# eth-ait/MultiPly

Measured on AMD Instinct MI355X. Metric: rays/sec rendering full 512x512 frames (eval forward, all persons, with background), higher is better.
Workload: dtype f16; 1 GPU; 2-person synthetic SMPL scene, 512x512 rays/frame, N_samples=128 (+32 extra +2 bounds = 161 composited samples/ray/person), N_samples_eval=128, 32 background samples, convergence groups of 512 rays (reference pixel_per_batch), geometric-init weights; frames=32, persons=2, sampler_sdf=bf16x3, parallelism=single GPU

## Files before the change

### multiply_amd/csrc/mlp.hip

```cpp
#include <hip/hip_runtime.h>
#include "common.hpp"
#include "../../include/multiply_hip.h"
#include "mlp_core.hpp"

using namespace mp;

namespace {

static_assert(sizeof(MpNet) == sizeof(NetDesc), "host / device net descriptors must match");
static_assert(MP_BIAS_STRIDE == BIAS_STRIDE && MP_MAX_LAYERS == MAX_LAYERS && MP_MAX_CHUNKS == MAX_CHUNKS, "abi");

constexpr int BIAS_BYTES = MAX_LAYERS * BIAS_STRIDE * 4;

template <int KS_IN, int NB, int WAVES>
struct Lds {
    static constexpr int PTS = 16 * NB;
    static constexpr int TILE = PTS * WAVES;
    static constexpr int ring = 0;
    static constexpr int bias0 = RING_SLOTS * chunk_bytes(KS_IN);
    static constexpr int bias1 = bias0 + BIAS_BYTES;
    static constexpr int stage = bias1 + BIAS_BYTES;
    static constexpr int scratch = stage + WAVES * PTS * in_stride(KS_IN) * 2;
    static constexpr int total = scratch + WAVES * PTS * 16;
};

template <int D, int L, int KS_IN>
__device__ __forceinline__ void stage_pe(op_t* row, const float (&x)[D]) {
    constexpr int NF = D + 2 * D * L;
    static_assert(NF <= KS_IN * 32, "encoding does not fit the input K steps");
#pragma unroll
    for (int a = 0; a < D; ++a) row[a] = (op_t)x[a];
#pragma unroll
    for (int a = 0; a < D; ++a) {
        float s, c;
        sincosf(x[a], &s, &c);
#pragma unroll
        for (int k = 0; k < L; ++k) {
            row[D + 2 * D * k + a] = (op_t)s;
            row[D + 2 * D * k + D + a] = (op_t)c;
            const float s2 = 2.0f * s * c, c2 = 1.0f - 2.0f * s * s;
            s = s2;
            c = c2;
        }
    }
#pragma unroll
    for (int f = NF; f < KS_IN * 32; ++f) row[f] = (op_t)0.0f;
}

template <int L, int KS_IN>
__device__ __forceinline__ void stage_pe_tangent(op_t* row, const float (&x)[3], int axis) {
    constexpr int D = 3;
#pragma unroll
    for (int f = 0; f < KS_IN * 32; ++f) row[f] = (op_t)0.0f;
    float s, c;
    const float xa = axis == 0 ? x[0] : (axis == 1 ? x[1] : x[2]);
    sincosf(xa, &s, &c);
    row[axis] = (op_t)TANGENT_SCALE;
    float f = TANGENT_SCALE;
#pragma unroll
    for (int k = 0; k < L; ++k) {
        row[D + 2 * D * k + axis] = (op_t)(f * c);
        row[D + 2 * D * k + D + axis] = (op_t)(-f * s);
        const float s2 = 2.0f * s * c, c2 = 1.0f - 2.0f * s * s;
        s = s2;
        c = c2;
        f *= 2.0f;
    }
}

template <int NB>
__device__ __forceinline__ void zero_b(opx8 (&B)[KS_REG][NB]) {
#pragma unroll
    for (int k = 0; k < KS_REG; ++k)
#pragma unroll
        for (int nb = 0; nb < NB; ++nb) B[k][nb] = (opx8)(op_t)0.0f;
}

template <int NB, int WAVES>
__global__ __launch_bounds__(WAVES * 64) void k_mlp_sdf(const NetDesc net, const char* __restrict__ wpack,
                                                        const float* __restrict__ bias, const float* __restrict__ xc,
                                                        const int* __restrict__ worklist,
                                                        const int* __restrict__ count_p, int max_count,
                                                        float* __restrict__ sdf_out) {
    constexpr int KS_IN = 2;
    using L = Lds<KS_IN, NB, WAVES>;
    extern __shared__ __attribute__((aligned(16))) char smem[];
    const int wave = threadIdx.x >> 6, lane = threadIdx.x & 63;
    const int count = count_p ? min(*count_p, max_count) : max_count;
    float* bias_lds = (float*)(smem + L::bias0);
    op_t* stage = (op_t*)(smem + L::stage) + wave * L::PTS * in_stride(KS_IN);
    load_bias(net, bias, bias_lds);
    for (int t = blockIdx.x; t * L::TILE < count; t += gridDim.x) {
        MP_STAMP_AT(HID_SOFTPLUS, 120, 0);
        prologue_issue<KS_IN, WAVES>(net, wpack, smem + L::ring, wave, lane);
        const int w = t * L::TILE + wave * L::PTS + lane;
        const int id = (lane < L::PTS && w < count) ? (worklist ? worklist[w] : w) : -1;
        if (lane < L::PTS) {
            float x[3] = {0.f, 0.f, 0.f};
            if (id >= 0) { x[0] = xc[3 * (size_t)id]; x[1] = xc[3 * (size_t)id + 1]; x[2] = xc[3 * (size_t)id + 2]; }
            stage_pe<3, 6, KS_IN>(stage + lane * in_stride(KS_IN), x);
        }
        MP_STAMP_AT(HID_SOFTPLUS, 120, 1);
        opx8 Bcur[KS_REG][NB];
        f32x4 out[NB];
        zero_b<NB>(Bcur);
        prologue_wait();
        MP_STAMP_AT(HID_SOFTPLUS, 120, 2);
        run_net<NB, false, KS_IN, HID_SOFTPLUS, WAVES>(net, wpack, bias_lds, smem + L::ring, Bcur, stage, out, wave, lane);
        MP_STAMP_AT(HID_SOFTPLUS, 120, 3);
#pragma unroll
        for (int nb = 0; nb < NB; ++nb) {
            const int pid = __shfl(id, nb * 16 + (lane & 15));
            if (lane < 16 && pid >= 0) sdf_out[pid] = out[nb][0];
        }
        MP_STAMP_AT(HID_SOFTPLUS, 121, 0);
    }
}

template <int WAVES>
__global__ __launch_bounds__(WAVES * 64) void k_mlp_sdf_x2(const NetDesc net, const char* __restrict__ wpack,
                                                           const float* __restrict__ bias, const float* __restrict__ xc,
                                                           const int* __restrict__ worklist,
                                                           const int* __restrict__ count_p, int max_count,
                                                           float* __restrict__ sdf_out) {
    constexpr int KS_IN = 2, NB = 2, WPTS = 16, TILE = WPTS * WAVES;
    using L = Lds<KS_IN, NB, WAVES>;
    constexpr int NF = 39, STR = in_stride(KS_IN);
    extern __shared__ __attribute__((aligned(16))) char smem[];
    const int wave = threadIdx.x >> 6, lane = threadIdx.x & 63, j = lane & 15, g = lane >> 4;
    const int count = count_p ? min(*count_p, max_count) : max_count;
    float* bias_lds = (float*)(smem + L::bias0);
    op_t* stage = (op_t*)(smem + L::stage) + wave * L::PTS * STR;
    load_bias(net, bias, bias_lds);
    for (int t = blockIdx.x; t * TILE < count; t += gridDim.x) {
        prologue_issue<KS_IN, WAVES>(net, wpack, smem + L::ring, wave, lane);
        const int w = t * TILE + wave * WPTS + j;
        const int id = w < count ? (worklist ? worklist[w] : w) : -1;
        {
            op_t* rh = stage + j * STR;
            op_t* rl = stage + (16 + j) * STR;
            auto put = [&](int f, float v) {
                const op_t hi = (op_t)v;
                rh[f] = hi;
                rl[f] = (op_t)(v - (float)hi);
            };
            if (g < 3) {
                const float x = id >= 0 ? xc[3 * (size_t)id + g] : 0.0f;
                put(g, x);
#pragma unroll
                for (int k = 0; k < 6; ++k) {
                    float sn, cs;
                    sincosf(x * (float)(1 << k), &sn, &cs);
                    put(3 + 6 * k + g, sn);
                    put(3 + 6 * k + 3 + g, cs);
                }
            } else {
#pragma unroll
                for (int f = NF; f < KS_IN * 32; ++f) { rh[f] = (op_t)0.0f; rl[f] = (op_t)0.0f; }
            }
        }
        opx8 Bcur[KS_REG][NB];
        f32x4 out[NB];
        zero_b<NB>(Bcur);
        prologue_wait();
        run_net<NB, false, KS_IN, HID_SOFTPLUS_X2, WAVES>(net, wpack, bias_lds, smem + L::ring, Bcur, stage, out, wave, lane);
        if (lane < 16 && id >= 0) sdf_out[id] = out[0][0] + out[1][0];
    }
}

template <int D_IN, int LFREQ, int KS_IN, int NB, int WAVES>
__global__ __launch_bounds__(WAVES * 64) void k_mlp_full(const NetDesc net, const char* __restrict__ wpack,
                                                         const float* __restrict__ bias, const float* __restrict__ x,
                                                         int n, float* __restrict__ outp) {
    using L = Lds<KS_IN, NB, WAVES>;
    extern __shared__ __attribute__((aligned(16))) char smem[];
    const int wave = threadIdx.x >> 6, lane = threadIdx.x & 63;
    float* bias_lds = (float*)(smem + L::bias0);
    op_t* stage = (op_t*)(smem + L::stage) + wave * L::PTS * in_stride(KS_IN);
    load_bias(net, bias, bias_lds);
    for (int t = blockIdx.x; t * L::TILE < n; t += gridDim.x) {
        const int id0 = t * L::TILE + wave * L::PTS;
        if (lane < L::PTS) {
            const int id = id0 + lane < n ? id0 + lane : -1;
            float xi[D_IN];
#pragma unroll
            for (int a = 0; a < D_IN; ++a) xi[a] = id >= 0 ? x[(size_t)id * D_IN + a] : 0.f;
            stage_pe<D_IN, LFREQ, KS_IN>(stage + lane * in_stride(KS_IN), xi);
        }
        opx8 Bcur[KS_REG][NB];
        f32x4 out[NB];
        zero_b<NB>(Bcur);
        prologue<KS_IN, WAVES>(net, wpack, smem + L::ring, wave, lane);
        run_net<NB, false, KS_IN, HID_SOFTPLUS, WAVES>(net, wpack, bias_lds, smem + L::ring, Bcur, stage, out, wave, lane);
        const int j = lane & 15, g = lane >> 4;
#pragma unroll
        for (int nb = 0; nb < NB; ++nb) {
            const int pid = id0 + nb * 16 + j;
            if (pid < n) {
                float* o = outp + (size_t)pid * 257;
                if (g == 0) o[0] = out[nb][0];
#pragma unroll
                for (int ks = 0; ks < KS_REG; ++ks)
#pragma unroll
                    for (int e = 0; e < 8; ++e)
                        o[1 + 32 * ks + (e < 4 ? 4 * g + e : 16 + 4 * g + e - 4)] = (float)Bcur[ks][nb][e];
            }
        }
    }
}

__global__ __launch_bounds__(512) void k_mlp_shade(const NetDesc net, const char* __restrict__ wpack,
                                                   const float* __restrict__ bias, const float* __restrict__ xc,
                                                   const float* __restrict__ jinv, const int* __restrict__ worklist,
                                                   const int* __restrict__ count_p, int max_count,
                                                   float* __restrict__ sdf_out, float* __restrict__ normal_out,
                                                   char* __restrict__ feat_frag) {
    constexpr int KS_IN = 2, NB = 2, WAVES = 8;
    using L = Lds<KS_IN, NB, WAVES>;
    extern __shared__ __attribute__((aligned(16))) char smem[];
    const int wave = threadIdx.x >> 6, lane = threadIdx.x & 63;
    const int count = count_p ? min(*count_p, max_count) : max_count;
    float* bias_lds = (float*)(smem + L::bias0);
    op_t* stage = (op_t*)(smem + L::stage) + wave * L::PTS * in_stride(KS_IN);
    load_bias(net, bias, bias_lds);
    for (int t = blockIdx.x; t * 64 < count; t += gridDim.x) {
        const int pt = lane & 7, role = 2 * ((lane >> 4) & 1) + ((lane >> 3) & 1);
        const int w = t * 64 + wave * 8 + pt;
        const int id = w < count ? (worklist ? worklist[w] : w) : -1;
        if (lane < 32) {
            float x[3] = {0.f, 0.f, 0.f};
            if (id >= 0) { x[0] = xc[3 * (size_t)id]; x[1] = xc[3 * (size_t)id + 1]; x[2] = xc[3 * (size_t)id + 2]; }
            op_t* row = stage + lane * in_stride(KS_IN);
            if (role == 0) stage_pe<3, 6, KS_IN>(row, x);
            else stage_pe_tangent<6, KS_IN>(row, x, role - 1);
        }
        opx8 Bcur[KS_REG][NB];
        f32x4 out[NB];
        zero_b<NB>(Bcur);
        prologue<KS_IN, WAVES, false>(net, wpack, smem + L::ring, wave, lane);
        run_net<NB, true, KS_IN, HID_SOFTPLUS, WAVES>(net, wpack, bias_lds, smem + L::ring, Bcur, stage, out, wave, lane);
        if ((lane & 8) == 0) {
            const int lp = ((lane & 15) + 8 * (wave & 1)) + 16 * (lane >> 4);
#pragma unroll
            for (int ks = 0; ks < KS_REG; ++ks)
                *(opx8*)(feat_frag + (((size_t)t * KS_REG + ks) * 4 + (wave >> 1)) * 1024 + lp * 16) = Bcur[ks][0];
        }
        constexpr float TS_INV = 1.0f / TANGENT_SCALE;
        const float gx = TS_INV * __shfl(out[0][0], (lane & 7) + 8), gz = TS_INV * __shfl(out[1][0], (lane & 7) + 8);
        if (lane < 8 && id >= 0) {
            const float gy = TS_INV * out[1][0];
            const float* Ji = jinv + 9 * (size_t)id;
            float n0 = gx * Ji[0] + gy * Ji[3] + gz * Ji[6];
            float n1 = gx * Ji[1] + gy * Ji[4] + gz * Ji[7];
            float n2 = gx * Ji[2] + gy * Ji[5] + gz * Ji[8];
            float inv = 1.0f / fmaxf(sqrtf(n0 * n0 + n1 * n1 + n2 * n2), 1e-12f);
            n0 *= inv; n1 *= inv; n2 *= inv;
            inv = 1.0f / fmaxf(sqrtf(n0 * n0 + n1 * n1 + n2 * n2), 1e-6f);
            sdf_out[id] = out[0][0];
            normal_out[3 * (size_t)id] = n0 * inv;
            normal_out[3 * (size_t)id + 1] = n1 * inv;
            normal_out[3 * (size_t)id + 2] = n2 * inv;
        }
    }
}

struct GradCapture {
    const op_t* tab_a;
    const op_t* tab_b;
    float (&g)[2][3];
    template <int NB>
    __device__ __forceinline__ void operator()(int cid, int bi, const f32x4 (&acc)[NB]) const {
        const int lane = threadIdx.x & 63, j = lane & 15, gq = lane >> 4;
        const op_t* tab = cid == 1 ? tab_a : tab_b;
#pragma unroll
        for (int nb = 0; nb < 2; ++nb) {
            const op_t* tp = tab + (16 * nb + j) * 48 + 16 * bi + 4 * gq;
#pragma unroll
            for (int r = 0; r < 4; ++r) {
                const float v = acc[nb][r] * (float)tp[r];
                const int k = (bi + r) % 3;
                g[nb][0] += k == 0 ? v : 0.0f;
                g[nb][1] += k == 1 ? v : 0.0f;
                g[nb][2] += k == 2 ? v : 0.0f;
            }
        }
    }
    static __device__ __forceinline__ void unrotate(float (&g)[2][3]) {
        const int s = ((threadIdx.x & 63) >> 4) % 3;
#pragma unroll
        for (int nb = 0; nb < 2; ++nb) {
            const float a0 = g[nb][0], a1 = g[nb][1], a2 = g[nb][2];
            g[nb][0] = s == 0 ? a0 : (s == 1 ? a2 : a1);
            g[nb][1] = s == 0 ? a1 : (s == 1 ? a0 : a2);
            g[nb][2] = s == 0 ? a2 : (s == 1 ? a1 : a0);
        }
    }
};


template <int NB, int WAVES>
__global__ __launch_bounds__(WAVES * 64) void k_mlp_fwdsave(const NetDesc net, const char* __restrict__ wpack,
                                                            const float* __restrict__ bias, const float* __restrict__ xc,
                                                            const int* __restrict__ worklist,
                                                            const int* __restrict__ count_p, int max_count, int offset,
                                                            int seg, float* __restrict__ sdf_out,
                                                            char* __restrict__ feat_frag, char* __restrict__ sigbuf) {
    constexpr int KS_IN = 2;
    using L = Lds<KS_IN, NB, WAVES>;
    static_assert(L::PTS == 32 && WAVES == 8, "feature / sigmoid block addressing assumes 8 waves x 32 points");
    extern __shared__ __attribute__((aligned(16))) char smem[];
    const int wave = threadIdx.x >> 6, lane = threadIdx.x & 63;
    const int count = min(count_p ? min(*count_p, max_count) : max_count, offset + seg);
    if (offset >= count) return;
    float* bias_lds = (float*)(smem + L::bias0);
    op_t* stage = (op_t*)(smem + L::stage) + wave * L::PTS * in_stride(KS_IN);
    load_bias(net, bias, bias_lds);
    constexpr int SIG_LAYER = KS_REG * SIG_CHUNK_BYTES;
    for (int t = blockIdx.x; offset + t * L::TILE < count; t += gridDim.x) {
        prologue_issue<KS_IN, WAVES>(net, wpack, smem + L::ring, wave, lane);
        const int w = offset + t * L::TILE + wave * L::PTS + lane;
        const int id = (lane < L::PTS && w < count) ? (worklist ? worklist[w] : w) : -1;
        if (lane < L::PTS) {
            float x[3] = {0.f, 0.f, 0.f};
            if (id >= 0) { x[0] = xc[3 * (size_t)id]; x[1] = xc[3 * (size_t)id + 1]; x[2] = xc[3 * (size_t)id + 2]; }
            stage_pe<3, 6, KS_IN>(stage + lane * in_stride(KS_IN), x);
        }
        opx8 Bcur[KS_REG][NB];
        f32x4 out[NB];
        zero_b<NB>(Bcur);
        prologue_wait();
        MP_STAMP_AT(HID_SOFTPLUS_SAVE, 120, 2);
        #ifdef MP_EXP_SIGCACHED
        const SigIO sio = {sigbuf + ((size_t)(blockIdx.x) * WAVES + wave) * (size_t)(8 * SIG_LAYER), SIG_LAYER};
#else
        const SigIO sio = {sigbuf + ((size_t)t * WAVES + wave) * (size_t)(8 * SIG_LAYER), SIG_LAYER};
#endif
        run_net<NB, false, KS_IN, HID_SOFTPLUS_SAVE, WAVES>(net, wpack, bias_lds, smem + L::ring, Bcur, stage, out, wave, lane,
                                                            sio);
        MP_STAMP_AT(HID_SOFTPLUS_SAVE, 120, 3);
        const size_t tile = (size_t)(offset / 64) + (size_t)t * 4 + (wave >> 1);
#pragma unroll
        for (int nb = 0; nb < NB; ++nb) {
#pragma unroll
            for (int ks = 0; ks < KS_REG; ++ks)
                *(opx8*)(feat_frag + ((tile * KS_REG + ks) * 4 + (wave & 1) * 2 + nb) * 1024 + lane * 16) = Bcur[ks][nb];
            const int pid = __shfl(id, nb * 16 + (lane & 15));
            if (lane < 16 && pid >= 0) sdf_out[pid] = out[nb][0];
        }
    }
}

template <int NB, int WAVES>
__global__ __launch_bounds__(WAVES * 64) void k_mlp_grad(const NetDesc net, const char* __restrict__ wpack,
                                                         const op_t* __restrict__ w8_slots, const float* __restrict__ xc,
                                                         const float* __restrict__ jinv, const int* __restrict__ worklist,
                                                         const int* __restrict__ count_p, int max_count, int offset, int seg,
                                                         const char* __restrict__ sigbuf, const float* __restrict__ sdf_in,
                                                         float* __restrict__ normal_out) {
    constexpr int KS_IN = 0, PTS = 16 * NB, TILE = PTS * WAVES;
    static_assert(NB == 2 && WAVES == 8, "matches k_mlp_fwdsave's tile / wave / point addressing");
    constexpr int RING = RING_SLOTS * chunk_bytes(KS_IN);
    extern __shared__ __attribute__((aligned(16))) char smem[];
    const int wave = threadIdx.x >> 6, lane = threadIdx.x & 63, gq = lane >> 4;
    const int count = min(count_p ? min(*count_p, max_count) : max_count, offset + seg);
    if (offset >= count) return;
    op_t* w8 = (op_t*)(smem + RING);
    op_t* tabs = w8 + 256 + wave * (2 * PTS * 48);
    for (int i = threadIdx.x; i < 256; i += blockDim.x) w8[i] = w8_slots[i];
    constexpr int SIG_LAYER = KS_REG * SIG_CHUNK_BYTES;
    for (int t = blockIdx.x; offset + t * TILE < count; t += gridDim.x) {
        const int w = offset + t * TILE + wave * PTS + (lane & (PTS - 1));
        const int id = w < count ? (worklist ? worklist[w] : w) : -1;
        if (lane < PTS) {
            float x[3] = {0.f, 0.f, 0.f};
            if (id >= 0) { x[0] = xc[3 * (size_t)id]; x[1] = xc[3 * (size_t)id + 1]; x[2] = xc[3 * (size_t)id + 2]; }
            op_t* ta = tabs + lane * 48;
            op_t* tb = tabs + PTS * 48 + lane * 48;
#pragma unroll
            for (int f = 0; f < 48; ++f) { ta[f] = (op_t)0.0f; tb[f] = (op_t)0.0f; }
#pragma unroll
            for (int a = 0; a < 3; ++a) {
                ta[a] = (op_t)1.0f;
                float sn, cs, fr = 1.0f;
                sincosf(x[a], &sn, &cs);
#pragma unroll
                for (int k = 0; k < 6; ++k) {
                    ta[3 + 6 * k + a] = (op_t)(fr * cs);
                    ta[3 + 6 * k + 3 + a] = (op_t)(-fr * sn);
                    const float s2 = 2.0f * sn * cs, c2 = 1.0f - 2.0f * sn * sn;
                    sn = s2; cs = c2; fr *= 2.0f;
                }
            }
#pragma unroll
            for (int f = 0; f < 39; ++f) tb[9 + f] = ta[f];
        }
        #ifdef MP_EXP_SIGCACHED
        const SigIO sio = {const_cast<char*>(sigbuf) + ((size_t)(blockIdx.x) * WAVES + wave) * (size_t)(8 * SIG_LAYER), SIG_LAYER};
#else
        const SigIO sio = {const_cast<char*>(sigbuf) + ((size_t)t * WAVES + wave) * (size_t)(8 * SIG_LAYER), SIG_LAYER};
#endif
        opx8 Bcur[KS_REG][NB];
        __syncthreads();
#pragma unroll
        for (int ks = 0; ks < KS_REG; ++ks) {
            const opx8 wv = *(const opx8*)(w8 + ks * 32 + 8 * gq);
            if constexpr (SIG8) {
                const u32x4 pk = *(const u32x4*)(sio.base + (size_t)7 * SIG_LAYER + ks * 1024 + lane * 16);
                const opx8 wq = wv * (op_t)SIG_QINV_F;
#pragma unroll
                for (int nb = 0; nb < NB; ++nb) {
                    const unsigned d0 = nb == 0 ? pk.x : pk.z, d1 = nb == 0 ? pk.y : pk.w;
                    u32x4 h;
                    h.x = __builtin_amdgcn_perm(0x64646464u, d0, 0x04010400u);
                    h.y = __builtin_amdgcn_perm(0x64646464u, d0, 0x04030402u);
                    h.z = __builtin_amdgcn_perm(0x64646464u, d1, 0x04010400u);
                    h.w = __builtin_amdgcn_perm(0x64646464u, d1, 0x04030402u);
                    Bcur[ks][nb] = (__builtin_bit_cast(opx8, h) - (op_t)1024.0f) * wq;
                }
            } else {
#pragma unroll
                for (int nb = 0; nb < NB; ++nb)
                    Bcur[ks][nb] = *(const opx8*)(sio.base + (size_t)7 * SIG_LAYER + (ks * NB + nb) * 1024 + lane * 16) * wv;
            }
        }
        float g[2][3] = {{0.f, 0.f, 0.f}, {0.f, 0.f, 0.f}};
        f32x4 out[NB];
#ifdef MP_EXP_GRAD_OLD
        prologue<KS_IN, WAVES, false>(net, wpack, smem, wave, lane);
#else
        prologue<KS_IN, WAVES>(net, wpack, smem, wave, lane);
#endif
        MP_STAMP_AT(HID_SIGMUL, 120, 2);
        run_net<NB, false, KS_IN, HID_SIGMUL, WAVES, GradCapture>(net, wpack, nullptr, smem, Bcur, nullptr, out, wave, lane, sio,
                                                                   GradCapture{tabs, tabs + PTS * 48, g});
        MP_STAMP_AT(HID_SIGMUL, 120, 3);
        GradCapture::unrotate(g);
#pragma unroll
        for (int nb = 0; nb < NB; ++nb)
#pragma unroll
            for (int a = 0; a < 3; ++a) {
                g[nb][a] += __shfl_xor(g[nb][a], 16);
                g[nb][a] += __shfl_xor(g[nb][a], 32);
            }
#pragma unroll
        for (int nb = 0; nb < NB; ++nb) {
            const int pid = __shfl(id, nb * 16 + (lane & 15));
            if (lane < 16 && pid >= 0) {
                const float gx = g[nb][0], gy = g[nb][1], gz = g[nb][2];
                const float* Ji = jinv + 9 * (size_t)pid;
                float n0 = gx * Ji[0] + gy * Ji[3] + gz * Ji[6];
                float n1 = gx * Ji[1] + gy * Ji[4] + gz * Ji[7];
                float n2 = gx * Ji[2] + gy * Ji[5] + gz * Ji[8];
                float inv = 1.0f / fmaxf(sqrtf(n0 * n0 + n1 * n1 + n2 * n2), 1e-12f);
                n0 *= inv; n1 *= inv; n2 *= inv;
                inv = 1.0f / fmaxf(sqrtf(n0 * n0 + n1 * n1 + n2 * n2), 1e-6f);
                const float poison = 0.0f * sdf_in[pid];
                normal_out[3 * (size_t)pid] = n0 * inv + poison;
                normal_out[3 * (size_t)pid + 1] = n1 * inv + poison;
                normal_out[3 * (size_t)pid + 2] = n2 * inv + poison;
            }
        }
        __syncthreads();
    }
}

template <int NB, int WAVES>
__global__ __launch_bounds__(WAVES * 64) void k_mlp_color(const NetDesc net, const char* __restrict__ wpack,
                                                          const float* __restrict__ bias, const float* __restrict__ xc,
                                                          const float* __restrict__ normal,
                                                          const char* __restrict__ feat_frag,
                                                          const int* __restrict__ worklist,
                                                          const int* __restrict__ count_p, int max_count,
                                                          float* __restrict__ rgb_out) {
    constexpr int KS_IN = 2;
    using L = Lds<KS_IN, NB, WAVES>;
    static_assert(64 % L::PTS == 0, "a wave consumes a whole number of column blocks of one 64-item shade tile");
    extern __shared__ __attribute__((aligned(16))) char smem[];
    const int wave = threadIdx.x >> 6, lane = threadIdx.x & 63;
    const int count = count_p ? min(*count_p, max_count) : max_count;
    float* bias_lds = (float*)(smem + L::bias0);
    op_t* stage = (op_t*)(smem + L::stage) + wave * L::PTS * in_stride(KS_IN);
    load_bias(net, bias, bias_lds);
    for (int t = blockIdx.x; t * L::TILE < count; t += gridDim.x) {
        MP_STAMP_AT(HID_RELU, 120, 0);
        const int w0 = t * L::TILE + wave * L::PTS;
        const int tile = w0 / 64, nb0 = (w0 % 64) / 16;
        const int w = w0 + lane;
        const int id = (lane < L::PTS && w < count) ? (worklist ? worklist[w] : w) : -1;
        prologue_issue<KS_IN, WAVES>(net, wpack, smem + L::ring, wave, lane);
        opx8 Bcur[KS_REG][NB];
        const bool live = w0 < count;
#pragma unroll
        for (int ks = 0; ks < KS_REG; ++ks)
#pragma unroll
            for (int nb = 0; nb < NB; ++nb)
                Bcur[ks][nb] = live ? *(const opx8*)(feat_frag + (((size_t)tile * KS_REG + ks) * 4 + nb0 + nb) * 1024 + lane * 16)
                                    : (opx8)(op_t)0.0f;
        if (lane < L::PTS) {
            op_t* row = stage + lane * in_stride(KS_IN);
#pragma unroll
            for (int f = 0; f < KS_IN * 32; ++f) row[f] = (op_t)0.0f;
            if (id >= 0) {
#pragma unroll
                for (int a = 0; a < 3; ++a) {
                    row[a] = (op_t)xc[3 * (size_t)id + a];
                    row[3 + a] = (op_t)normal[3 * (size_t)id + a];
                }
            }
        }
        MP_STAMP_AT(HID_RELU, 120, 1);
        f32x4 out[NB];
        prologue_wait();
        MP_STAMP_AT(HID_RELU, 120, 2);
        run_net<NB, false, KS_IN, HID_RELU, WAVES>(net, wpack, bias_lds, smem + L::ring, Bcur, stage, out, wave, lane);
        MP_STAMP_AT(HID_RELU, 120, 3);
#pragma unroll
        for (int nb = 0; nb < NB; ++nb) {
            const int pid = __shfl(id, nb * 16 + (lane & 15));
            if (lane < 16 && pid >= 0) {
                const float* nq = normal + 3 * (size_t)pid;
                const float poison = 0.0f * (nq[0] + nq[1] + nq[2]);
#pragma unroll
                for (int c = 0; c < 3; ++c) rgb_out[3 * (size_t)pid + c] = 1.0f / (1.0f + __expf(-out[nb][c])) + poison;
            }
        }
        MP_STAMP_AT(HID_RELU, 121, 0);
    }
}

template <int NB, int WAVES>
__global__ __launch_bounds__(WAVES * 64) void k_background(const NetDesc net_imp, const char* __restrict__ wp_imp,
                                                           const float* __restrict__ bias_imp, const NetDesc net_ren,
                                                           const char* __restrict__ wp_ren,
                                                           const float* __restrict__ bias_ren,
                                                           const float* __restrict__ dirs, const float* __restrict__ cam,
                                                           const float* __restrict__ z_bg, int z_per_ray, int n_rays,
                                                           float radius, float* __restrict__ bg_rgb) {
    constexpr int KS_IN = 3, NBG = 32;
    using L = Lds<KS_IN, NB, WAVES>;
    static_assert(L::PTS % NBG == 0, "whole rays per wave");
    extern __shared__ __attribute__((aligned(16))) char smem[];
    const int wave = threadIdx.x >> 6, lane = threadIdx.x & 63;
    float* bias_lds0 = (float*)(smem + L::bias0);
    float* bias_lds1 = (float*)(smem + L::bias1);
    op_t* stage = (op_t*)(smem + L::stage) + wave * L::PTS * in_stride(KS_IN);
    float* scr = (float*)(smem + L::scratch) + wave * L::PTS * 4;
    load_bias(net_imp, bias_imp, bias_lds0);
    load_bias(net_ren, bias_ren, bias_lds1);
    const int n_pts = n_rays * NBG;
    const float ox = cam[0], oy = cam[1], oz = cam[2];
    for (int t = blockIdx.x; t * L::TILE < n_pts; t += gridDim.x) {
        prologue_issue<KS_IN, WAVES>(net_imp, wp_imp, smem + L::ring, wave, lane);
        const int q = t * L::TILE + wave * L::PTS + lane;
        const int ray = q / NBG, s = q % NBG;
        float d[3] = {0.f, 0.f, 1.f};
        if (lane < L::PTS) {
            const bool ok = ray < n_rays;
            float depth = 0.1f;
            if (ok) {
                d[0] = dirs[3 * ray]; d[1] = dirs[3 * ray + 1]; d[2] = dirs[3 * ray + 2];
                depth = z_per_ray ? z_bg[(size_t)ray * NBG + s] : z_bg[s];
            }
            const float o_dot_d = d[0] * ox + d[1] * oy + d[2] * oz;
            const float under = o_dot_d * o_dot_d - ((ox * ox + oy * oy + oz * oz) - radius * radius);
            const float d_sphere = sqrtf(under) - o_dot_d;
            const float ps[3] = {ox + d_sphere * d[0], oy + d_sphere * d[1], oz + d_sphere * d[2]};
            const float pm[3] = {ox - o_dot_d * d[0], oy - o_dot_d * d[1], oz - o_dot_d * d[2]};
            const float pm_n = sqrtf(pm[0] * pm[0] + pm[1] * pm[1] + pm[2] * pm[2]);
            float ax[3] = {oy * ps[2] - oz * ps[1], oz * ps[0] - ox * ps[2], ox * ps[1] - oy * ps[0]};
            const float an = sqrtf(ax[0] * ax[0] + ax[1] * ax[1] + ax[2] * ax[2]);
            ax[0] /= an; ax[1] /= an; ax[2] /= an;
            const float phi = asinf(pm_n / radius), theta = asinf(pm_n * depth);
            float sa, ca;
            sincosf(phi - theta, &sa, &ca);
            const float cr[3] = {ax[1] * ps[2] - ax[2] * ps[1], ax[2] * ps[0] - ax[0] * ps[2], ax[0] * ps[1] - ax[1] * ps[0]};
            const float adp = ax[0] * ps[0] + ax[1] * ps[1] + ax[2] * ps[2];
            float pn[3];
#pragma unroll
            for (int a = 0; a < 3; ++a) pn[a] = ps[a] * ca + cr[a] * sa + ax[a] * adp * (1.0f - ca);
            const float pnn = sqrtf(pn[0] * pn[0] + pn[1] * pn[1] + pn[2] * pn[2]);
            const float x4[4] = {pn[0] / pnn, pn[1] / pnn, pn[2] / pnn, depth};
            stage_pe<4, 10, KS_IN>(stage + lane * in_stride(KS_IN), x4);
        }
        opx8 Bcur[KS_REG][NB];
        f32x4 out[NB];
        zero_b<NB>(Bcur);
        prologue_wait();
        run_net<NB, false, KS_IN, HID_SOFTPLUS, WAVES>(net_imp, wp_imp, bias_lds0, smem + L::ring, Bcur, stage, out, wave,
                                                       lane);
        prologue_issue<KS_IN, WAVES>(net_ren, wp_ren, smem + L::ring, wave, lane);
        if (lane < 16) {
#pragma unroll
            for (int nb = 0; nb < NB; ++nb) scr[(nb * 16 + lane) * 4 + 3] = fabsf(out[nb][0]);
        }
        if (lane < L::PTS) stage_pe<3, 4, KS_IN>(stage + lane * in_stride(KS_IN), d);
        prologue_wait();
        run_net<NB, false, KS_IN, HID_RELU, WAVES>(net_ren, wp_ren, bias_lds1, smem + L::ring, Bcur, stage, out, wave, lane);
        if (lane < 16) {
#pragma unroll
            for (int nb = 0; nb < NB; ++nb)
#pragma unroll
                for (int c = 0; c < 3; ++c) scr[(nb * 16 + lane) * 4 + c] = 1.0f / (1.0f + __expf(-out[nb][c]));
        }
        __syncthreads();
        if (lane < L::PTS / NBG) {
            const int r = (t * L::TILE + wave * L::PTS) / NBG + lane;
            if (r < n_rays) {
                float acc[3] = {0.f, 0.f, 0.f}, csum = 0.0f;
                for (int i = 0; i < NBG; ++i) {
                    const float zi = z_per_ray ? z_bg[(size_t)r * NBG + i] : z_bg[i];
                    const float zn = i + 1 < NBG ? (z_per_ray ? z_bg[(size_t)r * NBG + i + 1] : z_bg[i + 1]) : 0.f;
                    const float dist = i + 1 < NBG ? zi - zn : 1e10f;
                    const float* sp = scr + (lane * NBG + i) * 4;
                    const float fe = dist * sp[3];
                    const float alpha = 1.0f - expf(-fe);
                    const float wgt = alpha * expf(-csum);
                    acc[0] += wgt * sp[0]; acc[1] += wgt * sp[1]; acc[2] += wgt * sp[2];
                    csum += fe;
                }
                bg_rgb[3 * r] = acc[0]; bg_rgb[3 * r + 1] = acc[1]; bg_rgb[3 * r + 2] = acc[2];
            }
        }
    }
}

int grid_for(int work_blocks, int per_cu) {
    const int cap = 256 * per_cu;
    return work_blocks < cap ? (work_blocks > 0 ? work_blocks : 1) : cap;
}

NetDesc as_desc(const MpNet* net) {
    NetDesc d;
    __builtin_memcpy(&d, net, sizeof(d));
    return d;
}

bool net_ok(const MpNet* net) {
    if (!net || net->n_layers < 1 || net->n_layers > MAX_LAYERS) return false;
    bool linear_seen = false;
    int chunks = 0;
    for (int l = 0; l < net->n_layers; ++l) {
        const auto& L = net->layer[l];
        if (L.n_chunk < 1 || L.n_chunk > MAX_CHUNKS) return false;
        if (L.act == ACT_NONE) linear_seen = true;
        else if (linear_seen) return false;
        chunks += L.n_chunk;
    }
    return chunks == net->total_chunks;
}

constexpr int PNB = 2, PWAVES = 8;

}

#ifdef MP_EXP_STAMP
extern "C" int mp_debug_stamps(void* dst_host) {
    return (int)hipMemcpyFromSymbol(dst_host, HIP_SYMBOL(mp::mp_stamps), sizeof(mp::mp_stamps));
}
#endif

extern "C" int mp_mlp_sdf(const MpNet* net, const void* wpack, const float* bias, const float* xc,
                          const int* worklist, const int* count, int max_count, float* sdf_out, void* stream) {
    if (max_count <= 0) return 0;
    if (!net_ok(net)) return -1;
    hipStream_t st = (hipStream_t)stream;
    using L = Lds<2, PNB, PWAVES>;
    MP_LDS_ATTR((k_mlp_sdf<PNB, PWAVES>), L::total);
    const NetDesc d = as_desc(net);
    hipLaunchKernelGGL((k_mlp_sdf<PNB, PWAVES>), dim3(grid_for((max_count + L::TILE - 1) / L::TILE, 1)),
                       dim3(PWAVES * 64), L::total, st, d, (const char*)wpack, bias, xc, worklist, count, max_count,
                       sdf_out);
    return (int)hipGetLastError();
}

extern "C" int mp_mlp_sdf_x2(const MpNet* net, const void* wpack, const float* bias, const float* xc,
                             const int* worklist, const int* count, int max_count, float* sdf_out, void* stream) {
    if (max_count <= 0) return 0;
    if (!net_ok(net)) return -1;
    hipStream_t st = (hipStream_t)stream;
    using L = Lds<2, PNB, PWAVES>;
    constexpr int TILE = 16 * PWAVES;
    MP_LDS_ATTR((k_mlp_sdf_x2<PWAVES>), L::total);
    const NetDesc d = as_desc(net);
    hipLaunchKernelGGL((k_mlp_sdf_x2<PWAVES>), dim3(grid_for((max_count + TILE - 1) / TILE, 1)), dim3(PWAVES * 64), L::total, st,
                       d, (const char*)wpack, bias, xc, worklist, count, max_count, sdf_out);
    return (int)hipGetLastError();
}

extern "C" int mp_mlp_full(const MpNet* net, const void* wpack, const float* bias, const float* x, int d_in, int n,
                           float* out, void* stream) {
    if (n <= 0) return 0;
    if (!net_ok(net)) return -1;
    hipStream_t st = (hipStream_t)stream;
    const NetDesc d = as_desc(net);
    if (d_in == 3) {
        using L = Lds<2, PNB, PWAVES>;
        MP_LDS_ATTR((k_mlp_full<3, 6, 2, PNB, PWAVES>), L::total);
        hipLaunchKernelGGL((k_mlp_full<3, 6, 2, PNB, PWAVES>), dim3(grid_for((n + L::TILE - 1) / L::TILE, 1)),
                           dim3(PWAVES * 64), L::total, st, d, (const char*)wpack, bias, x, n, out);
    } else if (d_in == 4) {
        using L = Lds<3, PNB, PWAVES>;
        MP_LDS_ATTR((k_mlp_full<4, 10, 3, PNB, PWAVES>), L::total);
        hipLaunchKernelGGL((k_mlp_full<4, 10, 3, PNB, PWAVES>), dim3(grid_for((n + L::TILE - 1) / L::TILE, 1)),
                           dim3(PWAVES * 64), L::total, st, d, (const char*)wpack, bias, x, n, out);
    } else {
        return -1;
    }
    return (int)hipGetLastError();
}

extern "C" int mp_sig_bytes_per_point(void) { return 8 * KS_REG * SIG_CHUNK_BYTES / 32; }

extern "C" int mp_mlp_shade_rev(const MpNet* net, const void* wpack, const float* bias, const MpNet* gnet, const void* gpack,
                                const void* w8_slots, const float* xc, const float* jinv, const int* worklist,
                                const int* count, int max_count, float* sdf_out, float* normal_out, void* feat_frag,
                                void* sig, int seg_points, void* stream) {
    if (max_count <= 0) return 0;
    if (seg_points < 256 || seg_points % 256) return -1;
    if (!net_ok(net) || !net_ok(gnet)) return -1;
    for (int l = 0; l < gnet->n_layers; ++l)
        if (gnet->layer[l].act == ACT_SIGMUL && gnet->layer[l].n_chunk != KS_REG) return -1;
    hipStream_t st = (hipStream_t)stream;
    using L = Lds<2, PNB, PWAVES>;
    constexpr int TILE = 16 * PNB * PWAVES;
    constexpr int LDS_G = RING_SLOTS * chunk_bytes(0) + 512 + PWAVES * 2 * 16 * PNB * 48 * 2;
    MP_LDS_ATTR((k_mlp_fwdsave<PNB, PWAVES>), L::total);
    MP_LDS_ATTR((k_mlp_grad<PNB, PWAVES>), LDS_G);
    const NetDesc d = as_desc(net), gd = as_desc(gnet);
    for (int off = 0; off < max_count; off += seg_points) {
        const int n = max_count - off < seg_points ? max_count - off : seg_points;
        const int grid = grid_for((n + TILE - 1) / TILE, 1);
        hipLaunchKernelGGL((k_mlp_fwdsave<PNB, PWAVES>), dim3(grid), dim3(PWAVES * 64), L::total, st, d, (const char*)wpack, bias,
                           xc, worklist, count, max_count, off, seg_points, sdf_out, (char*)feat_frag, (char*)sig);
        hipLaunchKernelGGL((k_mlp_grad<PNB, PWAVES>), dim3(grid), dim3(PWAVES * 64), LDS_G, st, gd, (const char*)gpack,
                           (const op_t*)w8_slots, xc, jinv, worklist, count, max_count, off, seg_points, (const char*)sig,
                           sdf_out, normal_out);
    }
    return (int)hipGetLastError();
}

extern "C" int mp_mlp_shade(const MpNet* net, const void* wpack, const float* bias, const float* xc,
                            const float* jinv, const int* worklist, const int* count, int max_count, float* sdf_out,
                            float* normal_out, void* feat_frag, void* stream) {
    if (max_count <= 0) return 0;
    if (!net_ok(net)) return -1;
    hipStream_t st = (hipStream_t)stream;
    const NetDesc d = as_desc(net);
    using L = Lds<2, 2, 8>;
    MP_LDS_ATTR((k_mlp_shade), L::total);
    hipLaunchKernelGGL(k_mlp_shade, dim3(grid_for((max_count + 63) / 64, 1)), dim3(512), L::total, st, d,
                       (const char*)wpack, bias, xc, jinv, worklist, count, max_count, sdf_out, normal_out,
                       (char*)feat_frag);
    return (int)hipGetLastError();
}

extern "C" int mp_mlp_color(const MpNet* net, const void* wpack, const float* bias, const float* xc,
                            const float* normal, const void* feat_frag, const int* worklist, const int* count,
                            int max_count, float* rgb_out, void* stream) {
    if (max_count <= 0) return 0;
    if (!net_ok(net)) return -1;
    hipStream_t st = (hipStream_t)stream;
    using L = Lds<2, PNB, PWAVES>;
    MP_LDS_ATTR((k_mlp_color<PNB, PWAVES>), L::total);
    const NetDesc d = as_desc(net);
    hipLaunchKernelGGL((k_mlp_color<PNB, PWAVES>), dim3(grid_for((max_count + L::TILE - 1) / L::TILE, 1)),
                       dim3(PWAVES * 64), L::total, st, d, (const char*)wpack, bias, xc, normal, (const char*)feat_frag,
                       worklist, count, max_count, rgb_out);
    return (int)hipGetLastError();
}

extern "C" int mp_background(const MpNet* net_imp, const void* wpack_imp, const float* bias_imp, const MpNet* net_ren,
                             const void* wpack_ren, const float* bias_ren, const float* dirs, const float* cam,
                             const float* z_bg, int z_per_ray, int n_rays, float radius, float* bg_rgb, void* stream) {
    if (n_rays <= 0) return 0;
    if (!net_ok(net_imp) || !net_ok(net_ren)) return -1;
    hipStream_t st = (hipStream_t)stream;
    using L = Lds<3, PNB, PWAVES>;
    MP_LDS_ATTR((k_background<PNB, PWAVES>), L::total);
    const NetDesc d0 = as_desc(net_imp), d1 = as_desc(net_ren);
    hipLaunchKernelGGL((k_background<PNB, PWAVES>), dim3(grid_for((n_rays * 32 + L::TILE - 1) / L::TILE, 1)),
                       dim3(PWAVES * 64), L::total, st, d0, (const char*)wpack_imp, bias_imp, d1, (const char*)wpack_ren,
                       bias_ren, dirs, cam, z_bg, z_per_ray, n_rays, radius, bg_rgb);
    return (int)hipGetLastError();
}
```

### multiply_amd/csrc/mlp_core.hpp

```cpp
#pragma once
#include <hip/hip_runtime.h>
#include <stdint.h>

namespace mp {

typedef _Float16 op_t;
typedef op_t opx8 __attribute__((ext_vector_type(8)));
typedef op_t h2 __attribute__((ext_vector_type(2)));
constexpr float TANGENT_SCALE = 0.0625f;
typedef float f32x4 __attribute__((ext_vector_type(4)));

constexpr int KS_REG = 8;
constexpr int TILE_BYTES = 1024;
constexpr int CHUNK_MB = 2;
constexpr int MAX_CHUNKS = 9;
constexpr int MAX_LAYERS = 10;
constexpr int BIAS_STRIDE = MAX_CHUNKS * 32;
__host__ __device__ constexpr int mb_bytes(int ks_in) { return (KS_REG + ks_in) * TILE_BYTES; }
__host__ __device__ constexpr int chunk_bytes(int ks_in) { return CHUNK_MB * mb_bytes(ks_in); }
constexpr int RING_SLOTS = 3;
__host__ __device__ constexpr int in_stride(int ks_in) { return ks_in * 32 + 8; }

enum Act : int { ACT_NONE = 0, ACT_SOFTPLUS = 1, ACT_RELU = 2, ACT_SIGMUL = 3 };

struct LayerDesc {
    int n_chunk;
    int use_reg;
    int use_in;
    int act;
    int out_chunk;
    int aux;
};

struct NetDesc {
    int n_layers;
    int total_chunks;
    LayerDesc layer[MAX_LAYERS];
};

__device__ __forceinline__ void lds_dma_16(const void* gsrc_uniform, unsigned lane_off, unsigned lds_base) {
    asm volatile("s_mov_b32 m0, %0\n\ts_nop 0\n\tglobal_load_lds_dwordx4 %1, %2" ::"s"(lds_base), "v"(lane_off), "s"(gsrc_uniform)
                 : "memory");
}
#ifdef MP_EXP_NOWAIT
__device__ __forceinline__ void dma_wait_all() {}
#else
__device__ __forceinline__ void dma_wait_all() { __builtin_amdgcn_s_waitcnt(0x0F70); }
#endif
__device__ __forceinline__ unsigned lds_offset(const void* p) { return (unsigned)(size_t)p; }
__device__ __forceinline__ const char* uniform_ptr(const char* p) {
    const size_t v = (size_t)p;
    return (const char*)(((size_t)(unsigned)__builtin_amdgcn_readfirstlane((int)(v >> 32)) << 32) |
                         (unsigned)__builtin_amdgcn_readfirstlane((int)v));
}

template <int KS_IN, int WAVES, int P0 = 0, int P1 = 99>
__device__ __forceinline__ void issue_chunk(const char* __restrict__ wpack, char* wring, int ci, int wave, int lane) {
    constexpr int CB = chunk_bytes(KS_IN);
    constexpr int NP = CB / TILE_BYTES;
    constexpr int NI = (NP + WAVES - 1) / WAVES;
    const int wave_u = __builtin_amdgcn_readfirstlane(wave), ci_u = __builtin_amdgcn_readfirstlane(ci);
    const char* src = uniform_ptr(wpack) + (size_t)ci_u * CB + wave_u * TILE_BYTES;
    const unsigned dst = __builtin_amdgcn_readfirstlane(lds_offset(wring)) + (ci_u % RING_SLOTS) * CB + wave_u * TILE_BYTES;
#pragma unroll
    for (int i = P0; i < (P1 < NI ? P1 : NI); ++i) {
        if (wave_u + WAVES * i < NP) lds_dma_16(src + WAVES * i * TILE_BYTES, lane * 16, dst + WAVES * i * TILE_BYTES);
    }
}

typedef unsigned int u32x4 __attribute__((ext_vector_type(4)));
#if !defined(MP_DMA_LATE) && !defined(MP_DMA_EARLY)
#define MP_DMA_EARLY 1
#endif
#ifdef MP_EXP_NOMFMA
#define MP_MFMA_F16(a, b, c, x, y, z) (c)
#else
#define MP_MFMA_F16(a, b, c, x, y, z) __builtin_amdgcn_mfma_f32_16x16x32_f16(a, b, c, x, y, z)
#endif

#ifdef MP_EXP_STAMP
__device__ unsigned long long mp_stamps[8 * 128 * 4];
#ifndef MP_STAMP_HID
#define MP_STAMP_HID -1
#endif
#define MP_STAMP_OK(hid) (MP_STAMP_HID < 0 || (hid) == MP_STAMP_HID)
#define MP_STAMP(ev) do { if (MP_STAMP_OK(HID) && blockIdx.x == 0 && lane == 0 && ci < 120) mp_stamps[((wave) * 128 + ci) * 4 + (ev)] = __builtin_amdgcn_s_memtime(); } while (0)
#define MP_STAMP_AT(hid, slot, ev) do { if (MP_STAMP_OK(hid) && blockIdx.x == 0 && (threadIdx.x & 63) == 0) mp_stamps[((threadIdx.x >> 6) * 128 + (slot)) * 4 + (ev)] = __builtin_amdgcn_s_memtime(); } while (0)
#else
#define MP_STAMP(ev)
#define MP_STAMP_AT(hid, slot, ev)
#endif

typedef float f32x2 __attribute__((ext_vector_type(2)));
__device__ __forceinline__ h2 to_h2(float a, float b) {
    return __builtin_convertvector((f32x2){a, b}, h2);
}
__device__ __forceinline__ unsigned bits(h2 v) { return __builtin_bit_cast(unsigned, v); }

template <int NB, bool IN_AGPR>
struct NextB {
    unsigned r[KS_REG][NB][4];
    __device__ __forceinline__ void put(int c, int nb, int half, int j, h2 v) {
        const unsigned u = bits(v);
        if constexpr (IN_AGPR) {
            asm("v_accvgpr_write_b32 %0, %1" : "=a"(r[c][nb][2 * half + j]) : "v"(u));
        } else {
            r[c][nb][2 * half + j] = u;
        }
    }
    __device__ __forceinline__ void put_sel(int c_rt, int nb, int half, int j, h2 v) {
        static_assert(!IN_AGPR, "put_sel: VGPR-resident only");
        const unsigned u = bits(v);
#pragma unroll
        for (int c = 0; c < KS_REG; ++c) r[c][nb][2 * half + j] = c == c_rt ? u : r[c][nb][2 * half + j];
    }
    __device__ __forceinline__ void zero() {
#pragma unroll
        for (int c = 0; c < KS_REG; ++c)
#pragma unroll
            for (int nb = 0; nb < NB; ++nb)
#pragma unroll
                for (int i = 0; i < 4; ++i) {
                    if constexpr (IN_AGPR) asm("v_accvgpr_write_b32 %0, 0" : "=a"(r[c][nb][i]));
                    else r[c][nb][i] = 0u;
                }
    }
    __device__ __forceinline__ opx8 get(int c, int nb) const {
        u32x4 v;
#pragma unroll
        for (int i = 0; i < 4; ++i) {
            if constexpr (IN_AGPR) {
                unsigned t;
                asm("v_accvgpr_read_b32 %0, %1" : "=v"(t) : "a"(r[c][nb][i]));
                v[i] = t;
            } else {
                v[i] = r[c][nb][i];
            }
        }
        return __builtin_bit_cast(opx8, v);
    }
};

enum Hidden : int { HID_SOFTPLUS = 0, HID_RELU = 1, HID_SOFTPLUS_SAVE = 2, HID_SIGMUL = 3, HID_SOFTPLUS_X2 = 4 };
struct SigIO {
    char* base;
    int layer_bytes;
};

__device__ __forceinline__ h2 exp2_h2(h2 x) {
    unsigned r;
    const unsigned xi = bits(x);
    asm("v_exp_f16_sdwa %0, %1 dst_sel:DWORD dst_unused:UNUSED_PAD src0_sel:WORD_0\n\ts_nop 0\n\t"
        "v_exp_f16_sdwa %0, %1 dst_sel:WORD_1 dst_unused:UNUSED_PRESERVE src0_sel:WORD_1"
        : "=&v"(r) : "v"(xi));
    return __builtin_bit_cast(h2, r);
}
__device__ __forceinline__ h2 exp2_neg_abs_h2(h2 x) {
    unsigned r;
    const unsigned xi = bits(x);
    asm("v_exp_f16_sdwa %0, -|%1| dst_sel:DWORD dst_unused:UNUSED_PAD src0_sel:WORD_0\n\ts_nop 0\n\t"
        "v_exp_f16_sdwa %0, -|%1| dst_sel:WORD_1 dst_unused:UNUSED_PRESERVE src0_sel:WORD_1"
        : "=&v"(r) : "v"(xi));
    return __builtin_bit_cast(h2, r);
}
__device__ __forceinline__ h2 log2_h2(h2 x) {
    unsigned r;
    const unsigned xi = bits(x);
    asm("v_log_f16_sdwa %0, %1 dst_sel:DWORD dst_unused:UNUSED_PAD src0_sel:WORD_0\n\ts_nop 0\n\t"
        "v_log_f16_sdwa %0, %1 dst_sel:WORD_1 dst_unused:UNUSED_PRESERVE src0_sel:WORD_1"
        : "=&v"(r) : "v"(xi));
    return __builtin_bit_cast(h2, r);
}
typedef short s16x2 __attribute__((ext_vector_type(2)));
__device__ __forceinline__ h2 relu_h2(h2 z) {
    return __builtin_bit_cast(h2, __builtin_elementwise_max(__builtin_bit_cast(s16x2, z), (s16x2){0, 0}));
}
__device__ __forceinline__ h2 softplus2(h2 z) {
#ifdef MP_EXP_NOTRANS
    return relu_h2(z) + z * (h2){(op_t)0.001f, (op_t)0.001f};
#else
    const h2 u = exp2_neg_abs_h2(z);
#ifdef MP_EXP_LOGTRANS
    return relu_h2(z) + log2_h2(u + (h2){(op_t)1.0f, (op_t)1.0f});
#else
    const h2 c1 = {(op_t)1.42459527f, (op_t)1.42459527f}, c2 = {(op_t)-0.58921265f, (op_t)-0.58921265f},
             c3 = {(op_t)0.16538905f, (op_t)0.16538905f};
    h2 t = __builtin_elementwise_fma(u, c3, c2);
    t = __builtin_elementwise_fma(t, u, c1);
    return __builtin_elementwise_fma(t, u, relu_h2(z));
#endif
#endif
}
__device__ __forceinline__ h2 row_shr8(h2 s) {
    unsigned d;
    const unsigned si = bits(s);
    asm("s_nop 1\n\tv_mov_b32_dpp %0, %1 row_shr:8 row_mask:0xf bank_mask:0xf" : "=v"(d) : "v"(si), "0"(si));
    return __builtin_bit_cast(h2, d);
}

template <int NB, bool FWD, int HID, bool HIDDEN, int q, typename NB_T>
__device__ __forceinline__ void act_piece(const f32x4 (&p)[NB], NB_T& Bn, int pc, int ph, u32x4 (&sg)[NB],
                                          const SigIO& sig, int sig_layer) {
    static_assert(NB == 2, "the MLP core is specialised for 2 column blocks per wave (2 waves per SIMD)");
    if constexpr (FWD) {
        if constexpr (q < 2) {
            h2 z = to_h2(p[0][2 * q], p[0][2 * q + 1]);
            h2 t = to_h2(p[1][2 * q], p[1][2 * q + 1]);
            if constexpr (HIDDEN) {
                const bool vl = (threadIdx.x & 8) == 0;
                const h2 h = softplus2(z);
#ifdef MP_EXP_NOTRANS
                const h2 s = z * (h2){(op_t)0.01f, (op_t)0.01f};
#else
                const h2 s = exp2_h2(z - h);
#endif
                const h2 sf = row_shr8(s);
                const h2 zt = z * sf;
                z = vl ? h : zt;
                t = t * sf;
            }
            if (pc < KS_REG) {
                Bn.put(pc, 0, ph, q, z);
                Bn.put(pc, 1, ph, q, t);
            }
        }
    } else {
        if constexpr (q < 4) {
            constexpr int nb = q / 2, j = q % 2;
            h2 z = to_h2(p[nb][2 * j], p[nb][2 * j + 1]);
            if constexpr (HIDDEN) {
                if constexpr (HID == HID_SOFTPLUS_SAVE) {
                    const h2 h = softplus2(z);
#ifdef MP_EXP_NOTRANS
                    const unsigned sv = bits(z * (h2){(op_t)0.01f, (op_t)0.01f});
#else
                    const unsigned sv = bits(exp2_h2(z - h));
#endif
                    if (ph == 0) { if (j == 0) sg[nb][0] = sv; else sg[nb][1] = sv; }
                    else { if (j == 0) sg[nb][2] = sv; else sg[nb][3] = sv; }
                    z = h;
                    if (ph == 1 && j == 1 && pc < KS_REG)
                        *(u32x4*)(sig.base + (size_t)sig_layer * sig.layer_bytes + (pc * NB + nb) * 1024 + (threadIdx.x & 63) * 16) = sg[nb];
                } else if constexpr (HID == HID_SIGMUL) {
                    const unsigned sv = ph == 0 ? (j == 0 ? sg[nb][0] : sg[nb][1]) : (j == 0 ? sg[nb][2] : sg[nb][3]);
                    z = z * __builtin_bit_cast(h2, sv);
                } else {
                    z = HID == HID_SOFTPLUS ? softplus2(z) : relu_h2(z);
                }
            }
            if (pc < KS_REG) Bn.put(pc, nb, ph, j, z);
        }
    }
}

template <int NB, bool FWD, int HID, bool HIDDEN, int q, typename NB_T>
__device__ __forceinline__ void act_from(const f32x4 (&p)[NB], NB_T& Bn, int pc, int ph, u32x4 (&sg)[NB],
                                         const SigIO& sig, int sig_layer) {
    act_piece<NB, FWD, HID, HIDDEN, q>(p, Bn, pc, ph, sg, sig, sig_layer);
    if constexpr (q + 1 < 8) act_from<NB, FWD, HID, HIDDEN, q + 1>(p, Bn, pc, ph, sg, sig, sig_layer);
}

constexpr int SIG_BUFS = 2;
template <int HID>
__device__ __forceinline__ constexpr int sig_slot(int pc) { return pc & 1; }

template <int NB, bool FWD, int HID, bool HIDDEN, typename NB_T>
__device__ __forceinline__ void act_drain(const f32x4 (&p)[NB], NB_T& Bn, int pc_rt, u32x4 (&sgb)[SIG_BUFS][NB],
                                          const SigIO& sig, int sig_layer) {
    const bool odd = pc_rt & 1;
#define MP_SG(nb, i) (odd ? sgb[1][nb][i] : sgb[0][nb][i])
    if constexpr (FWD) {
#pragma unroll
        for (int q = 0; q < 2; ++q) {
            h2 z = to_h2(p[0][2 * q], p[0][2 * q + 1]);
            h2 t = to_h2(p[1][2 * q], p[1][2 * q + 1]);
            if constexpr (HIDDEN) {
                const bool vl = (threadIdx.x & 8) == 0;
                const h2 h = softplus2(z);
                const h2 s = exp2_h2(z - h);
                const h2 sf = row_shr8(s);
                const h2 zt = z * sf;
                z = vl ? h : zt;
                t = t * sf;
            }
            Bn.put_sel(pc_rt, 0, 1, q, z);
            Bn.put_sel(pc_rt, 1, 1, q, t);
        }
    } else {
#pragma unroll
        for (int nb = 0; nb < NB; ++nb) {
            const unsigned s0 = MP_SG(nb, 0), s1 = MP_SG(nb, 1);
            unsigned s2 = MP_SG(nb, 2), s3 = MP_SG(nb, 3);
            h2 z0 = to_h2(p[nb][0], p[nb][1]), z1 = to_h2(p[nb][2], p[nb][3]);
            if constexpr (HIDDEN) {
                if constexpr (HID == HID_SOFTPLUS_SAVE) {
                    const h2 h0 = softplus2(z0), h1 = softplus2(z1);
                    s2 = bits(exp2_h2(z0 - h0));
                    s3 = bits(exp2_h2(z1 - h1));
                    z0 = h0;
                    z1 = h1;
                } else if constexpr (HID == HID_SIGMUL) {
                    z0 = z0 * __builtin_bit_cast(h2, s2);
                    z1 = z1 * __builtin_bit_cast(h2, s3);
                } else {
                    z0 = HID == HID_SOFTPLUS ? softplus2(z0) : relu_h2(z0);
                    z1 = HID == HID_SOFTPLUS ? softplus2(z1) : relu_h2(z1);
                }
            }
            Bn.put_sel(pc_rt, nb, 1, 0, z0);
            Bn.put_sel(pc_rt, nb, 1, 1, z1);
            if constexpr (HIDDEN && HID == HID_SOFTPLUS_SAVE) {
                if (pc_rt < KS_REG)
                    *(u32x4*)(sig.base + (size_t)sig_layer * sig.layer_bytes + (pc_rt * NB + nb) * 1024 + (threadIdx.x & 63) * 16) =
                        (u32x4){s0, s1, s2, s3};
            }
        }
    }
#undef MP_SG
}

constexpr int A_PF = 3, A_QN = 4;
#ifndef MP_PP_PF
#define MP_PP_PF 3
#endif
constexpr int PP_PF = MP_PP_PF, PP_QN = PP_PF + 1;
constexpr int AQ_LEN = PP_QN > A_QN ? PP_QN : A_QN;
struct ActRegs8 {
    unsigned z[8], u[8], lg[8], r[8], h[8], d[8], s[8];
};
#ifdef MP_EXP_LOGTRANS
constexpr bool LOG_POLY = false;
#else
constexpr bool LOG_POLY = true;
#endif
constexpr float LOG2P_C1 = 1.42459527f, LOG2P_C2 = -0.58921265f, LOG2P_C3 = 0.16538905f;
#ifdef MP_EXP_SIG16
constexpr bool SIG8 = false;
#else
constexpr bool SIG8 = true;
#endif
#ifndef MP_EXP_SIGBITS
#define MP_EXP_SIGBITS 8
#endif
constexpr unsigned SIG_Q = MP_EXP_SIGBITS == 4 ? 0x4B804B80u : MP_EXP_SIGBITS == 6 ? 0x53E053E0u : 0x5BF85BF8u;
constexpr unsigned SIG_QINV = MP_EXP_SIGBITS == 4 ? 0x2C442C44u : MP_EXP_SIGBITS == 6 ? 0x24102410u : 0x1C041C04u;
constexpr unsigned SIG_Q_INT = MP_EXP_SIGBITS == 4 ? 15u : MP_EXP_SIGBITS == 6 ? 63u : 255u;
constexpr float SIG_QINV_F = MP_EXP_SIGBITS == 4 ? 1.0f / 15.0f : MP_EXP_SIGBITS == 6 ? 1.0f / 63.0f : 1.0f / 255.0f;
constexpr int SIG_CHUNK_BYTES = SIG8 ? 1024 : 2048;
#ifdef MP_SIG_FROM_H
constexpr bool SIG_FROM_H = SIG8;
#else
constexpr bool SIG_FROM_H = false;
#endif
struct ActConst {
    unsigned c1, c2, c3;
    unsigned c1024, c64;
    unsigned ctop;
};
__device__ __forceinline__ ActConst act_const() {
    const h2 a = {(op_t)LOG2P_C1, (op_t)LOG2P_C1}, b = {(op_t)LOG2P_C2, (op_t)LOG2P_C2}, c = {(op_t)LOG2P_C3, (op_t)LOG2P_C3};
    const h2 k = {(op_t)1024.0f, (op_t)1024.0f};
    return ActConst{bits(a), bits(b), bits(c), bits(k), 0x64646464u, 0x64006400u + (SIG_Q_INT | (SIG_Q_INT << 16))};
}
__device__ __forceinline__ unsigned sconst(unsigned v) { return (unsigned)__builtin_amdgcn_readfirstlane((int)v); }
__host__ __device__ constexpr int pp_stages(int hid, bool hidden) {
    return !hidden ? 1 : hid == HID_SOFTPLUS_SAVE ? (LOG_POLY ? 10 : 11) + (SIG8 ? 2 : 0) - (SIG_FROM_H ? 1 : 0) : hid == HID_SOFTPLUS ? (LOG_POLY ? 7 : 8)
                     : hid == HID_SIGMUL && SIG8 ? 5 : 2;
}

template <int HID, bool HIDDEN, int ST, int q, typename NB_T>
__device__ __forceinline__ void pp_instr(ActRegs8& a, const ActConst& k, const f32x4 (&acc)[CHUNK_MB][2], NB_T& Bn, int c,
                                         u32x4 (&sg)[2]) {
    constexpr int mbl = q / 4, nb = (q / 2) % 2, j = q % 2;
    constexpr bool SP = HIDDEN && (HID == HID_SOFTPLUS || HID == HID_SOFTPLUS_SAVE);
    constexpr int E0 = 1, E1 = 2, P0 = LOG_POLY ? 3 : -1, P1 = LOG_POLY ? 4 : -1, A1 = LOG_POLY ? -1 : 3, L0 = LOG_POLY ? -1 : 4,
                  L1 = LOG_POLY ? -1 : 5, RL = LOG_POLY ? 5 : 6, HH = LOG_POLY ? 6 : 7, SB = SIG_FROM_H ? -1 : HH + 1,
                  S0 = SIG_FROM_H ? HH + 1 : HH + 2, S1 = S0 + 1;
    if constexpr (ST == 0) {
        a.z[q] = bits(to_h2(acc[mbl][nb][2 * j], acc[mbl][nb][2 * j + 1]));
        if constexpr (!HIDDEN) {
            if (c < KS_REG) Bn.put(c, nb, mbl, j, __builtin_bit_cast(h2, a.z[q]));
        }
    } else if constexpr (HID == HID_SIGMUL && SIG8) {
        static_assert(ST >= 1 && ST <= 4 && HIDDEN, "pp_instr: stage");
        constexpr int e = 2 * nb + mbl;
        if constexpr (ST == 1) {
            unsigned src;
            if constexpr (e == 0) src = sg[0].x;
            else if constexpr (e == 1) src = sg[0].y;
            else if constexpr (e == 2) src = sg[0].z;
            else src = sg[0].w;
            asm volatile("v_perm_b32 %0, %1, %2, %3" : "=v"(a.u[q]) : "v"(k.c64), "v"(src), "s"(sconst(j == 0 ? 0x04010400u : 0x04030402u)));
        } else if constexpr (ST == 2) {
            asm volatile("v_pk_add_f16 %0, %0, %1 neg_lo:[0,1] neg_hi:[0,1]" : "+v"(a.u[q]) : "v"(k.c1024));
        } else if constexpr (ST == 3) {
            asm volatile("v_pk_mul_f16 %0, %0, %1" : "+v"(a.u[q]) : "s"(sconst(SIG_QINV)));
        } else {
            const h2 z = __builtin_bit_cast(h2, a.z[q]) * __builtin_bit_cast(h2, a.u[q]);
            if (c < KS_REG) Bn.put(c, nb, mbl, j, z);
        }
    } else if constexpr (!SP) {
        static_assert(ST == 1 && HIDDEN, "pp_instr: stage");
        h2 z = __builtin_bit_cast(h2, a.z[q]);
        if constexpr (HID == HID_SIGMUL) {
            constexpr int e = 2 * mbl + j;
            unsigned sv;
            if constexpr (e == 0) sv = sg[nb].x;
            else if constexpr (e == 1) sv = sg[nb].y;
            else if constexpr (e == 2) sv = sg[nb].z;
            else sv = sg[nb].w;
            z = z * __builtin_bit_cast(h2, sv);
        } else {
            z = relu_h2(z);
        }
        if (c < KS_REG) Bn.put(c, nb, mbl, j, z);
    } else if constexpr (ST == E0) {
        asm volatile("v_exp_f16_sdwa %0, -|%1| dst_sel:DWORD dst_unused:UNUSED_PAD src0_sel:WORD_0" : "=v"(a.u[q]) : "v"(a.z[q]));
    } else if constexpr (ST == E1) {
        asm volatile("v_exp_f16_sdwa %0, -|%1| dst_sel:WORD_1 dst_unused:UNUSED_PRESERVE src0_sel:WORD_1" : "+v"(a.u[q]) : "v"(a.z[q]));
    } else if constexpr (ST == P0) {
        asm volatile("v_pk_fma_f16 %0, %1, %2, %3" : "=v"(a.lg[q]) : "v"(a.u[q]), "v"(k.c3), "v"(k.c2));
    } else if constexpr (ST == P1) {
        asm volatile("v_pk_fma_f16 %0, %0, %1, %2" : "+v"(a.lg[q]) : "v"(a.u[q]), "v"(k.c1));
    } else if constexpr (ST == A1) {
        asm volatile("v_pk_add_f16 %0, %0, 1.0 op_sel_hi:[1,0]" : "+v"(a.u[q]));
    } else if constexpr (ST == L0) {
        asm volatile("v_log_f16_sdwa %0, %1 dst_sel:DWORD dst_unused:UNUSED_PAD src0_sel:WORD_0" : "=&v"(a.lg[q]) : "v"(a.u[q]));
    } else if constexpr (ST == L1) {
        asm volatile("v_log_f16_sdwa %0, %1 dst_sel:WORD_1 dst_unused:UNUSED_PRESERVE src0_sel:WORD_1" : "+v"(a.lg[q]) : "v"(a.u[q]));
    } else if constexpr (ST == RL) {
        asm volatile("v_pk_max_i16 %0, %1, 0" : "=v"(a.r[q]) : "v"(a.z[q]));
    } else if constexpr (ST == HH) {
        if constexpr (LOG_POLY) asm volatile("v_pk_fma_f16 %0, %1, %2, %3" : "=v"(a.h[q]) : "v"(a.lg[q]), "v"(a.u[q]), "v"(a.r[q]));
        else asm volatile("v_pk_add_f16 %0, %1, %2" : "=v"(a.h[q]) : "v"(a.r[q]), "v"(a.lg[q]));
        if (c < KS_REG) Bn.put(c, nb, mbl, j, __builtin_bit_cast(h2, a.h[q]));
    } else if constexpr (ST == SB) {
        asm volatile("v_pk_add_f16 %0, %1, %2 neg_lo:[0,1] neg_hi:[0,1]" : "=v"(a.d[q]) : "v"(a.z[q]), "v"(a.h[q]));
    } else if constexpr (ST == S0) {
        if constexpr (SIG_FROM_H)
            asm volatile("v_exp_f16_sdwa %0, -%1 dst_sel:DWORD dst_unused:UNUSED_PAD src0_sel:WORD_0" : "=&v"(a.s[q]) : "v"(a.h[q]));
        else
            asm volatile("v_exp_f16_sdwa %0, %1 dst_sel:DWORD dst_unused:UNUSED_PAD src0_sel:WORD_0" : "=&v"(a.s[q]) : "v"(a.d[q]));
    } else if constexpr (ST == S1) {
        if constexpr (SIG_FROM_H)
            asm volatile("v_exp_f16_sdwa %0, -%1 dst_sel:WORD_1 dst_unused:UNUSED_PRESERVE src0_sel:WORD_1" : "+v"(a.s[q]) : "v"(a.h[q]));
        else
            asm volatile("v_exp_f16_sdwa %0, %1 dst_sel:WORD_1 dst_unused:UNUSED_PRESERVE src0_sel:WORD_1" : "+v"(a.s[q]) : "v"(a.d[q]));
        if constexpr (!SIG8) {
            constexpr int e = 2 * mbl + j;
            if constexpr (e == 0) sg[nb].x = a.s[q];
            else if constexpr (e == 1) sg[nb].y = a.s[q];
            else if constexpr (e == 2) sg[nb].z = a.s[q];
            else sg[nb].w = a.s[q];
        }
    } else if constexpr (ST == S1 + 1) {
        static_assert(SIG8, "pp_instr: stage");
        if constexpr (SIG_FROM_H)
            asm volatile("v_pk_fma_f16 %0, %0, %1, %2" : "+v"(a.s[q]) : "s"(sconst(SIG_Q | 0x80008000u)), "v"(k.ctop));
        else
            asm volatile("v_pk_fma_f16 %0, %0, %1, %2" : "+v"(a.s[q]) : "s"(sconst(SIG_Q)), "v"(k.c1024));
    } else {
        static_assert(SIG8 && ST == S1 + 2, "pp_instr: stage");
        if constexpr (j == 0) {
            unsigned d;
            asm volatile("v_perm_b32 %0, %1, %2, %3" : "=v"(d) : "v"(a.s[q + 1]), "v"(a.s[q]), "s"(sconst(0x06040200u)));
            constexpr int e = 2 * nb + mbl;
            if constexpr (e == 0) sg[0].x = d;
            else if constexpr (e == 1) sg[0].y = d;
            else if constexpr (e == 2) sg[0].z = d;
            else sg[0].w = d;
        }
    }
}
template <int HID, bool HIDDEN, int I, typename NB_T>
__device__ __forceinline__ void pp_program(ActRegs8& a, const ActConst& k, const f32x4 (&acc)[CHUNK_MB][2], NB_T& Bn, int c,
                                           u32x4 (&sg)[2]) {
    if constexpr (I < 8 * pp_stages(HID, HIDDEN)) {
        pp_instr<HID, HIDDEN, I / 8, I % 8>(a, k, acc, Bn, c, sg);
        pp_program<HID, HIDDEN, I + 1>(a, k, acc, Bn, c, sg);
    }
}

template <typename NB_T>
__device__ __forceinline__ void x2_program(const f32x4 (&acc)[CHUNK_MB][2], NB_T& Bn, int c) {
    float h[8];
#pragma unroll
    for (int q = 0; q < 8; ++q) {
        const float z = acc[q >> 2][0][q & 3] + acc[q >> 2][1][q & 3];
        const float u = __builtin_amdgcn_exp2f(-__builtin_fabsf(z));
        h[q] = __builtin_fmaxf(z, 0.0f) + __builtin_amdgcn_logf(1.0f + u);
    }
#pragma unroll
    for (int p = 0; p < 4; ++p) {
        const h2 hi = to_h2(h[2 * p], h[2 * p + 1]);
        const h2 lo = to_h2(h[2 * p] - (float)hi[0], h[2 * p + 1] - (float)hi[1]);
        if (c < KS_REG) {
            Bn.put(c, 0, p >> 1, p & 1, hi);
            Bn.put(c, 1, p >> 1, p & 1, lo);
        }
    }
}

struct ChunkMasks {
    unsigned long long reg[2], in[2];
    __device__ __forceinline__ bool has_reg(int ci) const { return ((ci < 64 ? reg[0] >> ci : reg[1] >> (ci - 64)) & 1ull) != 0; }
    __device__ __forceinline__ bool has_in(int ci) const { return ((ci < 64 ? in[0] >> ci : in[1] >> (ci - 64)) & 1ull) != 0; }
};
__device__ __forceinline__ unsigned long long uniform_u64(unsigned long long v) {
    return ((unsigned long long)(unsigned)__builtin_amdgcn_readfirstlane((int)(v >> 32)) << 32) |
           (unsigned)__builtin_amdgcn_readfirstlane((int)v);
}
__device__ __forceinline__ ChunkMasks chunk_masks(const NetDesc& net) {
    unsigned long long r0 = 0, r1 = 0, i0 = 0, i1 = 0;
    int ci = 0;
    for (int l = 0; l < net.n_layers; ++l) {
        const int n = net.layer[l].n_chunk;
        const unsigned long long run = (1ull << n) - 1ull;
        const unsigned long long lo = ci < 64 ? run << ci : 0ull;
        const unsigned long long hi = ci >= 64 ? run << (ci - 64) : (ci + n > 64 ? run >> (64 - ci) : 0ull);
        if (net.layer[l].use_reg) { r0 |= lo; r1 |= hi; }
        if (net.layer[l].use_in) { i0 |= lo; i1 |= hi; }
        ci += n;
    }
    return ChunkMasks{{uniform_u64(r0), uniform_u64(r1)}, {uniform_u64(i0), uniform_u64(i1)}};
}

template <int KS_IN>
struct DmaLanes {
    unsigned reg[4];
    unsigned in[(2 * KS_IN + 3) / 4 + 1];
    unsigned run;
    unsigned wl;
};
template <int KS_IN>
__device__ __forceinline__ DmaLanes<KS_IN> dma_lanes(int wl, int lane) {
    DmaLanes<KS_IN> d;
    d.wl = wl;
    d.run = lane * 16 + (wl >> 1) * mb_bytes(KS_IN) + (wl & 1) * 4 * TILE_BYTES;
#pragma unroll
    for (int i = 0; i < 4; ++i) d.reg[i] = lane * 16 + (i / 2) * mb_bytes(KS_IN) + (wl + 4 * (i % 2)) * TILE_BYTES;
    if constexpr (KS_IN > 0) {
#pragma unroll
        for (int i = 0; i < (2 * KS_IN + 3) / 4; ++i) {
            const int k = wl + 4 * i;
            d.in[i] = lane * 16 + (k / KS_IN) * mb_bytes(KS_IN) + (KS_REG + k % KS_IN) * TILE_BYTES;
        }
    }
    return d;
}
__device__ __forceinline__ void pp_dma_piece(const char* src_chunk_uniform, unsigned lane_off, unsigned lds_chunk_base,
                                             unsigned piece_off_uniform) {
#ifdef MP_EXP_DMA1LANE
    asm volatile("s_mov_b64 s[98:99], exec\n\ts_mov_b64 exec, 1\n\ts_add_u32 m0, %0, %1\n\ts_nop 0\n\tglobal_load_lds_dwordx4 %2, %3\n\t"
                 "s_mov_b64 exec, s[98:99]"
                 ::"s"(lds_chunk_base), "s"(piece_off_uniform), "v"(lane_off), "s"(src_chunk_uniform) : "memory", "s98", "s99");
#else
    asm volatile("s_add_u32 m0, %0, %1\n\ts_nop 0\n\tglobal_load_lds_dwordx4 %2, %3"
                 ::"s"(lds_chunk_base), "s"(piece_off_uniform), "v"(lane_off), "s"(src_chunk_uniform) : "memory");
#endif
}
template <int KS_IN, int PART = 0>
__device__ __forceinline__ void pp_issue(const char* __restrict__ wpack, char* wring, int cn, int ring_slot,
                                         const ChunkMasks& cm, const DmaLanes<KS_IN>& d) {
    constexpr int CB = chunk_bytes(KS_IN);
    const int cn_u = __builtin_amdgcn_readfirstlane(cn);
    const char* src = uniform_ptr(wpack) + (size_t)cn_u * CB;
    const unsigned dst = __builtin_amdgcn_readfirstlane(lds_offset(wring)) + __builtin_amdgcn_readfirstlane(ring_slot) * CB;
    const unsigned wl = __builtin_amdgcn_readfirstlane(d.wl);
    if (cm.has_reg(cn_u)) {
#ifdef MP_DMA_ONE_M0
        const unsigned run = (wl >> 1) * mb_bytes(KS_IN) + (wl & 1) * 4 * TILE_BYTES;
        asm volatile("s_add_u32 m0, %0, %1\n\ts_nop 0\n\tglobal_load_lds_dwordx4 %2, %3\n\tglobal_load_lds_dwordx4 %2, %3 offset:1024\n\t"
                     "global_load_lds_dwordx4 %2, %3 offset:2048\n\tglobal_load_lds_dwordx4 %2, %3 offset:3072"
                     ::"s"(dst), "s"(run), "v"(d.run), "s"(src) : "memory");
#else
#pragma unroll
        for (int i = 0; i < 4; ++i)
            if (PART == 0 || i / 2 == PART - 1)
                pp_dma_piece(src, d.reg[i], dst, (i / 2) * mb_bytes(KS_IN) + (wl + 4 * (i % 2)) * TILE_BYTES);
#endif
    }
    if constexpr (KS_IN > 0) {
        if (cm.has_in(cn_u)) {
#pragma unroll
            for (int i = 0; i < (2 * KS_IN + 3) / 4; ++i) {
                const unsigned k = wl + 4 * i;
                if (k < 2 * KS_IN && (PART == 0 || k / KS_IN == PART - 1))
                    pp_dma_piece(src, d.in[i], dst, (k / KS_IN) * mb_bytes(KS_IN) + (KS_REG + k % KS_IN) * TILE_BYTES);
            }
        }
    }
}

struct NoCapture {
    template <int NB>
    __device__ __forceinline__ void operator()(int, int, const f32x4 (&)[NB]) const {}
};

template <int KS_IN, int HID, int WAVES, bool HIDDEN, typename Cap, typename NB_T>
__device__ __forceinline__ void run_layer_pp(const NetDesc& net, const LayerDesc L, int l, const char* __restrict__ wpack,
                                             const float* bias_lds, char* wring, opx8 (&Bcur)[KS_REG][2], NB_T& Bn,
                                             opx8 (&aq)[AQ_LEN], u32x4 (&sgb)[SIG_BUFS][2], const op_t* stage_wave,
                                             f32x4 (&out)[2], int wave, int lane, const SigIO& sig, Cap& cap, int& ci,
                                             int& ring_pos, const ChunkMasks& cm, const DmaLanes<KS_IN>& dl, int pp_last) {
    constexpr int PF = PP_PF, QN = PP_QN, NT = 2 * KS_REG;
    constexpr bool BIAS = HID != HID_SIGMUL;
    const int g = lane >> 4;
    const float* bl = BIAS ? bias_lds + l * BIAS_STRIDE + g * 4 : nullptr;
    const int sig_layer = HID == HID_SIGMUL ? (L.aux & 0xff) - 1 : l;
    const int cap_id = (L.aux >> 8) & 0xff;
    const bool late = __builtin_amdgcn_readfirstlane(wave) >= WAVES / 2;
    const ActConst kact = act_const();
#pragma unroll
    for (int c = 0; c < MAX_CHUNKS; ++c) {
        if ((HIDDEN ? c < KS_REG : true) && c < L.n_chunk) {
            MP_STAMP(0);
            const int ring_next = ring_pos + 1 == RING_SLOTS ? 0 : ring_pos + 1;
            const char* slot = wring + ring_pos * chunk_bytes(KS_IN) + lane * 16;
            const char* slot_next = wring + ring_next * chunk_bytes(KS_IN) + lane * 16;
            constexpr bool REV = HID == HID_SIGMUL && HIDDEN;
#ifdef MP_EXP_NOAHEAD
            constexpr bool AHEAD = false;
#else
            constexpr bool AHEAD = REV;
#endif
            u32x4 (&sg)[2] = sgb[0];
            u32x4 sgn[2];
            constexpr int SGV = SIG8 ? 1 : 2;
            if constexpr (REV) {
                if (!AHEAD || c == 0) {
#pragma unroll
                    for (int v = 0; v < SGV; ++v)
                        sg[v] = *(const u32x4*)(sig.base + (size_t)sig_layer * sig.layer_bytes + (c * SGV + v) * 1024 + lane * 16);
                }
                if (AHEAD && c + 1 < KS_REG) {
#pragma unroll
                    for (int v = 0; v < SGV; ++v)
                        sgn[v] = *(const u32x4*)(sig.base + (size_t)sig_layer * sig.layer_bytes + ((c + 1) * SGV + v) * 1024 + lane * 16);
                }
            }
            f32x4 acc[CHUNK_MB][2];
#pragma unroll
            for (int mbl = 0; mbl < CHUNK_MB; ++mbl) {
                f32x4 bv = (f32x4){0, 0, 0, 0};
                if constexpr (BIAS) bv = *(const f32x4*)(bl + (2 * c + mbl) * 16);
                acc[mbl][0] = bv;
                acc[mbl][1] = HID == HID_SOFTPLUS_X2 ? (f32x4){0, 0, 0, 0} : bv;
            }
            if (L.use_reg) {
#pragma unroll
                for (int t = 0; t < NT; ++t) {
                    const int ks = t / 2, mbl = t % 2;
                    const opx8 a = aq[t % QN];
#ifndef MP_EXP_NOLDS
                    if (t + PF < NT) {
                        const int tn = t + PF;
                        aq[tn % QN] = *(const opx8*)(slot + (tn % 2) * mb_bytes(KS_IN) + (tn / 2) * TILE_BYTES);
                    }
#endif
                    __builtin_amdgcn_sched_barrier(0);
#pragma unroll
                    for (int nb = 0; nb < 2; ++nb)
                        acc[mbl][nb] = MP_MFMA_F16(a, Bcur[ks][nb], acc[mbl][nb], 0, 0, 0);
                    __builtin_amdgcn_sched_barrier(0);
                }
            }
            if constexpr (KS_IN > 0) {
                if (L.use_in) {
#pragma unroll
                    for (int ks = 0; ks < KS_IN; ++ks) {
                        opx8 bi[2];
#pragma unroll
                        for (int nb = 0; nb < 2; ++nb)
                            bi[nb] = *(const opx8*)(stage_wave + (nb * 16 + (lane & 15)) * in_stride(KS_IN) + ks * 32 + g * 8);
#pragma unroll
                        for (int mbl = 0; mbl < CHUNK_MB; ++mbl) {
                            const opx8 a = *(const opx8*)(slot + mbl * mb_bytes(KS_IN) + (KS_REG + ks) * TILE_BYTES);
#pragma unroll
                            for (int nb = 0; nb < 2; ++nb)
                                acc[mbl][nb] = MP_MFMA_F16(a, bi[nb], acc[mbl][nb], 0, 0, 0);
                        }
                    }
                }
            }
            if (cap_id == 1) {
                if (c == 0) { cap(1, 0, acc[0]); cap(1, 1, acc[1]); }
                else if (c == 1) cap(1, 2, acc[0]);
            } else if (cap_id == 2) {
                if (c == 6) cap(2, 0, acc[1]);
                else if (c == 7) { cap(2, 1, acc[0]); cap(2, 2, acc[1]); }
            }
            if constexpr (!HIDDEN) {
                if (c == 0 || c == MAX_CHUNKS - 1) {
                    if (c == L.out_chunk) {
#pragma unroll
                        for (int nb = 0; nb < 2; ++nb) out[nb] = acc[0][nb];
                    }
                }
            }
            MP_STAMP(1);
            if constexpr (REV) {
                if (AHEAD && c + 1 < KS_REG) __builtin_amdgcn_s_waitcnt(0x0F70 | SGV);
                else dma_wait_all();
            }
            if (late) {
#if defined(MP_DMA_SPLIT)
                if constexpr (!REV) dma_wait_all();
                __syncthreads();
                if (ci + 3 <= pp_last) pp_issue<KS_IN, 2>(wpack, wring, ci + 3, ring_pos, cm, dl);
#elif defined(MP_DMA_EARLY)
                __syncthreads();
#else
                if constexpr (!REV) dma_wait_all();
                __syncthreads();
#ifndef MP_EXP_NOLOAD
                if (ci + 3 <= pp_last) pp_issue<KS_IN>(wpack, wring, ci + 3, ring_pos, cm, dl);
#endif
#endif
                MP_STAMP(2);
            }
            __builtin_amdgcn_sched_barrier(0);
            {
                ActRegs8 a;
#ifdef MP_EXP_NOV
                asm volatile("" ::"v"(acc[0][0]), "v"(acc[0][1]), "v"(acc[1][0]), "v"(acc[1][1]));
#else
                if constexpr (HID == HID_SOFTPLUS_X2) {
                    if constexpr (HIDDEN) x2_program(acc, Bn, c);
                } else {
                    pp_program<HID, HIDDEN, 0>(a, kact, acc, Bn, c, sg);
                }
#endif
                if constexpr (HID == HID_SOFTPLUS_SAVE && HIDDEN) {
#pragma unroll
                    for (int v = 0; v < SGV; ++v)
                        *(u32x4*)(sig.base + (size_t)sig_layer * sig.layer_bytes + (c * SGV + v) * 1024 + lane * 16) = sg[v];
                }
            }
            __builtin_amdgcn_sched_barrier(0);
            if constexpr (REV) {
                if (AHEAD && c + 1 < KS_REG) {
#pragma unroll
                    for (int v = 0; v < SGV; ++v) sg[v] = sgn[v];
                }
            }
            if (!late) {
                MP_STAMP(2);
#ifdef MP_DMA_EARLY
                if constexpr (HID == HID_SOFTPLUS_SAVE && HIDDEN) __builtin_amdgcn_s_waitcnt(0x0F70 | (SIG8 ? 1 : 2));
                else if constexpr (!REV) dma_wait_all();
#ifndef MP_EXP_NOLOAD
#ifdef MP_DMA_SPLIT
                if (ci >= 1 && ci + 2 <= pp_last)
                    pp_issue<KS_IN, 1>(wpack, wring, ci + 2, ring_pos == 0 ? RING_SLOTS - 1 : ring_pos - 1, cm, dl);
#else
                if (ci >= 1 && ci + 2 <= pp_last)
                    pp_issue<KS_IN>(wpack, wring, ci + 2, ring_pos == 0 ? RING_SLOTS - 1 : ring_pos - 1, cm, dl);
#endif
#endif
#endif
                __syncthreads();
            }
            MP_STAMP(3);
#pragma unroll
            for (int t = 0; t < PF; ++t)
                aq[t % QN] = *(const opx8*)(slot_next + (t % 2) * mb_bytes(KS_IN) + (t / 2) * TILE_BYTES);
            ++ci;
            ring_pos = ring_next;
        }
    }
#pragma unroll
    for (int k = 0; k < KS_REG; ++k)
#pragma unroll
        for (int nb = 0; nb < 2; ++nb) Bcur[k][nb] = Bn.get(k, nb);
}


__device__ __forceinline__ constexpr int act_shift(int hid) { return hid == HID_SIGMUL ? 4 : 0; }

template <int NB, bool FWD, int KS_IN, int HID, int WAVES, bool HIDDEN, typename Cap, typename NB_T>
__device__ __forceinline__ void run_layer(const NetDesc& net, const LayerDesc L, int l, const char* __restrict__ wpack,
                                          const float* bias_lds, char* wring, opx8 (&Bcur)[KS_REG][NB], NB_T& Bn,
                                          opx8 (&aq)[AQ_LEN], u32x4 (&sgb)[SIG_BUFS][NB], const op_t* stage_wave,
                                          f32x4 (&out)[NB], int wave, int lane, const SigIO& sig, Cap& cap, int& ci) {
    constexpr int PF = A_PF, QN = A_QN;
    constexpr bool BIAS = HID != HID_SIGMUL;
    const int g = lane >> 4;
    const float* bl = BIAS ? bias_lds + l * BIAS_STRIDE + g * 4 : nullptr;
    const int sig_layer = HID == HID_SIGMUL ? (L.aux & 0xff) - 1 : l;
    const int cap_id = (L.aux >> 8) & 0xff;
    f32x4 accs[2][NB];
    f32x4 bv_next = (f32x4){0, 0, 0, 0};
    if constexpr (BIAS) bv_next = *(const f32x4*)bl;
    auto load_sig = [&](int cc) {
#pragma unroll
        for (int nb = 0; nb < NB; ++nb)
            sgb[sig_slot<HID>(cc)][nb] = *(const u32x4*)(sig.base + (size_t)sig_layer * sig.layer_bytes + (cc * NB + nb) * 1024 +
                                                         lane * 16);
    };
#pragma unroll
    for (int c = 0; c < MAX_CHUNKS; ++c) {
        if (c < L.n_chunk) {
            MP_STAMP(0);
#ifndef MP_EXP_DMA_FIRST
            if constexpr (HID == HID_SIGMUL && HIDDEN) load_sig(c);
#endif
#if !defined(MP_EXP_NOLOAD) && !defined(MP_EXP_SPREAD_DMA)
            if (ci + 2 < net.total_chunks) issue_chunk<KS_IN, WAVES>(wpack, wring, ci + 2, wave, lane);
#endif
#ifdef MP_EXP_DMA_FIRST
            if constexpr (HID == HID_SIGMUL && HIDDEN) load_sig(c);
#endif
            const char* slot = wring + (ci % RING_SLOTS) * chunk_bytes(KS_IN) + lane * 16;
            const char* slot_next = wring + ((ci + 1) % RING_SLOTS) * chunk_bytes(KS_IN) + lane * 16;
#pragma unroll
            for (int mbl = 0; mbl < CHUNK_MB; ++mbl) {
#ifdef MP_EXP_PRIO
                if (((wave >> 2) ^ mbl) & 1) __builtin_amdgcn_s_setprio(1); else __builtin_amdgcn_s_setprio(0);
#endif
#ifdef MP_EXP_SPREAD_DMA
                if (ci + 2 < net.total_chunks) {
                    if (mbl == 0) issue_chunk<KS_IN, WAVES, 0, 1>(wpack, wring, ci + 2, wave, lane);
                    else issue_chunk<KS_IN, WAVES, 1, 99>(wpack, wring, ci + 2, wave, lane);
                }
#endif
                f32x4 (&acc)[NB] = accs[mbl];
                const f32x4 (&pend)[NB] = accs[mbl ^ 1];
                const f32x4 bv = bv_next;
                if constexpr (BIAS) bv_next = *(const f32x4*)(bl + (2 * c + mbl + 1) * 16);
#pragma unroll
                for (int nb = 0; nb < NB; ++nb) acc[nb] = (FWD && nb > 0) ? (f32x4){0, 0, 0, 0} : bv;
                if constexpr (FWD) {
                    if (threadIdx.x & 8) acc[0] = (f32x4){0, 0, 0, 0};
                }
                const char* tile = slot + mbl * mb_bytes(KS_IN);
                const bool has_pend = mbl == 1 || c > 0;
                const int pc = mbl == 1 ? c : c - 1, ph = mbl == 1 ? 0 : 1;
#ifdef MP_EXP_NOACT
#define MP_ACT_STMT(KS)
#else
#define MP_ACT_STMT(KS)                                                                                               \
    if constexpr (KS >= act_shift(HID)) {                                                                             \
        if (has_pend)                                                                                                 \
            act_piece<NB, FWD, HID, HIDDEN, KS - act_shift(HID)>(pend, Bn, pc, ph, sgb[sig_slot<HID>(pc)], sig, sig_layer); \
    }
#endif
#ifdef MP_EXP_NOLDS
#define MP_LDS_STMT (void)src;
#else
#define MP_LDS_STMT aq[nk % QN] = *(const opx8*)src;
#endif
#define MP_QSKIP(KS)                                                                                                  \
    {                                                                                                                 \
        constexpr int nk = KS + PF;                                                                                   \
        const char* src = nk < KS_REG ? tile + nk * TILE_BYTES                                                        \
                          : (mbl + 1 < CHUNK_MB ? tile + mb_bytes(KS_IN) + (nk - KS_REG) * TILE_BYTES                 \
                                                : slot_next + (nk - KS_REG) * TILE_BYTES);                            \
        if (nk >= KS_REG) { MP_LDS_STMT }                                                                             \
    }
#define MP_KSTEP(KS)                                                                                                  \
    {                                                                                                                 \
        const opx8 a = aq[KS % QN];                                                                                 \
        {                                                                                                             \
            constexpr int nk = KS + PF;                                                                               \
            const char* src = nk < KS_REG ? tile + nk * TILE_BYTES                                                    \
                              : (mbl + 1 < CHUNK_MB ? tile + mb_bytes(KS_IN) + (nk - KS_REG) * TILE_BYTES             \
                                                    : slot_next + (nk - KS_REG) * TILE_BYTES);                        \
            MP_LDS_STMT                                                                                               \
        }                                                                                                             \
        _Pragma("unroll") for (int nb = 0; nb < NB; ++nb)                                                             \
            acc[nb] = MP_MFMA_F16(a, Bcur[KS][nb], acc[nb], 0, 0, 0);                     \
        MP_ACT_STMT(KS)                                                                                               \
        __builtin_amdgcn_sched_group_barrier(0x100, 1, 0);                                                            \
        _Pragma("unroll") for (int q = 0; q < NB; ++q) {                                                              \
            __builtin_amdgcn_sched_group_barrier(0x008, 1, 0);                                                        \
            __builtin_amdgcn_sched_group_barrier(0x002, 5, 0);                                                        \
        }                                                                                                             \
        __builtin_amdgcn_sched_barrier(0);                                                                            \
    }
                if (L.use_reg) {
                    MP_KSTEP(0) MP_KSTEP(1) MP_KSTEP(2) MP_KSTEP(3) MP_KSTEP(4) MP_KSTEP(5) MP_KSTEP(6) MP_KSTEP(7)
                } else {
                    MP_QSKIP(0) MP_QSKIP(1) MP_QSKIP(2) MP_QSKIP(3) MP_QSKIP(4) MP_QSKIP(5) MP_QSKIP(6) MP_QSKIP(7)
#ifndef MP_EXP_NOACT
                    if (has_pend) act_from<NB, FWD, HID, HIDDEN, 0>(pend, Bn, pc, ph, sgb[sig_slot<HID>(pc)], sig, sig_layer);
#endif
                }
#undef MP_KSTEP
#undef MP_QSKIP
#undef MP_ACT_STMT
#undef MP_LDS_STMT
                if (L.use_in) {
#pragma unroll
                    for (int ks = 0; ks < KS_IN; ++ks) {
                        const opx8 a = *(const opx8*)(tile + (KS_REG + ks) * TILE_BYTES);
#pragma unroll
                        for (int nb = 0; nb < NB; ++nb) {
                            const opx8 bi = *(const opx8*)(stage_wave + (nb * 16 + (lane & 15)) * in_stride(KS_IN) +
                                                               ks * 32 + g * 8);
                            acc[nb] = MP_MFMA_F16(a, bi, acc[nb], 0, 0, 0);
                        }
                    }
                }
                if (cap_id == 1) {
                    if (c == 0) cap(1, mbl, acc);
                    else if (c == 1 && mbl == 0) cap(1, 2, acc);
                } else if (cap_id == 2) {
                    if (c == 6 && mbl == 1) cap(2, 0, acc);
                    else if (c == 7) cap(2, 1 + mbl, acc);
                }
                if ((c == 0 || c == MAX_CHUNKS - 1) && mbl == 0) {
                    if (c == L.out_chunk) {
#pragma unroll
                        for (int nb = 0; nb < NB; ++nb) out[nb] = acc[nb];
                    }
                }
            }
            MP_STAMP(1);
#ifndef MP_EXP_NOBARRIER
            dma_wait_all();
            MP_STAMP(2);
            __syncthreads();
            MP_STAMP(3);
#endif
            ++ci;
        }
    }
    act_drain<NB, FWD, HID, HIDDEN>(accs[1], Bn, L.n_chunk - 1, sgb, sig, sig_layer);
#pragma unroll
    for (int k = 0; k < KS_REG; ++k)
#pragma unroll
        for (int nb = 0; nb < NB; ++nb) Bcur[k][nb] = Bn.get(k, nb);
}

template <int NB, bool FWD, int KS_IN, int HID, int WAVES, typename Cap = NoCapture>
__device__ __forceinline__ void run_net(const NetDesc& net, const char* __restrict__ wpack, const float* bias_lds,
                                        char* wring, opx8 (&Bcur)[KS_REG][NB], const op_t* stage_wave,
                                        f32x4 (&out)[NB], int wave, int lane, SigIO sig = SigIO{nullptr, 0},
                                        Cap cap = Cap()) {
    int ci = 0;
    u32x4 sgb[SIG_BUFS][NB];
#pragma unroll
    for (int b = 0; b < SIG_BUFS; ++b)
#pragma unroll
        for (int nb = 0; nb < NB; ++nb) sgb[b][nb] = (u32x4){0u, 0u, 0u, 0u};
    NextB<NB, false> Bn;
    Bn.zero();
    opx8 aq[AQ_LEN];
#pragma unroll
    for (int t = 0; t < A_PF; ++t) aq[t] = *(const opx8*)(wring + t * TILE_BYTES + lane * 16);
    int l = 0;
#ifdef MP_EXP_NOPP
    constexpr bool PP = false;
#else
#ifdef MP_EXP_GRAD_OLD
    constexpr bool PP = !FWD && NB == 2 && HID != HID_SIGMUL;
#else
    constexpr bool PP = !FWD && NB == 2;
#endif
#endif
    static_assert(PP || !SIG8 || (HID != HID_SOFTPLUS_SAVE && HID != HID_SIGMUL),
                  "the interleaved (round-1) stream stores half-precision sigmoids: build the ablation with -DMP_EXP_SIG16");
    if constexpr (PP) {
        const int pp_last = net.total_chunks - 1;
        const ChunkMasks cm = chunk_masks(net);
        const DmaLanes<KS_IN> dl = dma_lanes<KS_IN>(__builtin_amdgcn_readfirstlane(wave) & (WAVES / 2 - 1), lane);
        int ring_pos = 0;
#pragma unroll
        for (int t = 0; t < PP_PF; ++t)
            aq[t % PP_QN] = *(const opx8*)(wring + (t % 2) * mb_bytes(KS_IN) + (t / 2) * TILE_BYTES + lane * 16);
        for (; l < net.n_layers && net.layer[l].act != ACT_NONE; ++l)
            run_layer_pp<KS_IN, HID, WAVES, true>(net, net.layer[l], l, wpack, bias_lds, wring, Bcur, Bn, aq, sgb, stage_wave, out,
                                                  wave, lane, sig, cap, ci, ring_pos, cm, dl, pp_last);
        for (; l < net.n_layers; ++l)
            run_layer_pp<KS_IN, HID, WAVES, false>(net, net.layer[l], l, wpack, bias_lds, wring, Bcur, Bn, aq, sgb, stage_wave, out,
                                                   wave, lane, sig, cap, ci, ring_pos, cm, dl, pp_last);
    }
    if constexpr (!PP) {
        for (; l < net.n_layers && net.layer[l].act != ACT_NONE; ++l)
            run_layer<NB, FWD, KS_IN, HID, WAVES, true>(net, net.layer[l], l, wpack, bias_lds, wring, Bcur, Bn, aq, sgb, stage_wave,
                                                        out, wave, lane, sig, cap, ci);
    }
    for (; l < net.n_layers; ++l)
        run_layer<NB, FWD, KS_IN, HID, WAVES, false>(net, net.layer[l], l, wpack, bias_lds, wring, Bcur, Bn, aq, sgb, stage_wave,
                                                     out, wave, lane, sig, cap, ci);
}

#ifdef MP_EXP_NOPP
constexpr bool PROLOGUE_THREE = false;
#else
constexpr bool PROLOGUE_THREE = true;
#endif
template <int KS_IN, int WAVES, bool THREE = PROLOGUE_THREE>
__device__ __forceinline__ void prologue_issue(const NetDesc& net, const char* __restrict__ wpack, char* wring, int wave, int lane) {
    issue_chunk<KS_IN, WAVES>(wpack, wring, 0, wave, lane);
    if (net.total_chunks > 1) issue_chunk<KS_IN, WAVES>(wpack, wring, 1, wave, lane);
    if constexpr (THREE) {
        if (net.total_chunks > 2) issue_chunk<KS_IN, WAVES>(wpack, wring, 2, wave, lane);
    }
}
__device__ __forceinline__ void prologue_wait() {
    dma_wait_all();
    __syncthreads();
}
template <int KS_IN, int WAVES, bool THREE = PROLOGUE_THREE>
__device__ __forceinline__ void prologue(const NetDesc& net, const char* __restrict__ wpack, char* wring, int wave,
                                         int lane) {
    prologue_issue<KS_IN, WAVES, THREE>(net, wpack, wring, wave, lane);
    prologue_wait();
}
__device__ __forceinline__ void load_bias(const NetDesc& net, const float* __restrict__ bias, float* bias_lds) {
    for (int i = threadIdx.x; i < net.n_layers * BIAS_STRIDE; i += blockDim.x) bias_lds[i] = bias[i];
}

}
```

Baseline: 2.854 million rays/s.

## Stream weight ring across tiles and prefetch next tile's inputs

The weight-chunk DMA ring now continues across tile iterations. When another tile follows, the last chunks of the current pass prefetch the first chunks of the next pass (or of the next network), so the per-tile prologue issue, wait and barrier are skipped. Each kernel also gets a TileInputs helper that loads worklist ids and coordinates one or two tiles ahead, hiding global-load latency. The cost is more complex ring-position bookkeeping and extra registers, which can hurt occupancy, plus a risk of ring or synchronisation hazards at tile boundaries.

```diff
diff --git a/multiply_amd/csrc/mlp.hip b/multiply_amd/csrc/mlp.hip
--- a/multiply_amd/csrc/mlp.hip
+++ b/multiply_amd/csrc/mlp.hip
@@ -68,6 +68,10 @@
     }
 }
 
+__device__ __forceinline__ float lane_value(float v, int lane_uniform) {
+    return __builtin_bit_cast(float, __builtin_amdgcn_readlane(__builtin_bit_cast(int, v), lane_uniform));
+}
+
 template <int NB>
 __device__ __forceinline__ void zero_b(opx8 (&B)[KS_REG][NB]) {
 #pragma unroll
@@ -75,6 +79,37 @@
 #pragma unroll
         for (int nb = 0; nb < NB; ++nb) B[k][nb] = (opx8)(op_t)0.0f;
 }
+
+template <int TILE>
+struct TileInputs {
+    const float* __restrict__ xc;
+    const int* __restrict__ worklist;
+    int base, count, slot, stride;
+    int id_next, id_after;
+    float x_next[3];
+    __device__ __forceinline__ int fetch_id(int t) const {
+        const long long w = (long long)base + (long long)t * TILE + slot;
+        return (slot >= 0 && w < count) ? (worklist ? worklist[w] : (int)w) : -1;
+    }
+    __device__ __forceinline__ void fetch_x(int id, float (&x)[3]) const {
+        x[0] = x[1] = x[2] = 0.0f;
+        if (id >= 0) { x[0] = xc[3 * (size_t)id]; x[1] = xc[3 * (size_t)id + 1]; x[2] = xc[3 * (size_t)id + 2]; }
+    }
+    __device__ __forceinline__ TileInputs(const float* xc_, const int* wl, int base_, int count_, int slot_, int t0, int stride_)
+        : xc(xc_), worklist(wl), base(base_), count(count_), slot(slot_), stride(stride_) {
+        id_next = fetch_id(t0);
+        id_after = fetch_id(t0 + stride);
+        fetch_x(id_next, x_next);
+    }
+    __device__ __forceinline__ int take(int t, float (&x)[3]) {
+        const int id = id_next;
+        x[0] = x_next[0]; x[1] = x_next[1]; x[2] = x_next[2];
+        id_next = id_after;
+        fetch_x(id_next, x_next);
+        id_after = fetch_id(t + 2 * stride);
+        return id;
+    }
+};
 
 template <int NB, int WAVES>
 __global__ __launch_bounds__(WAVES * 64) void k_mlp_sdf(const NetDesc net, const char* __restrict__ wpack,
@@ -90,30 +125,32 @@
     float* bias_lds = (float*)(smem + L::bias0);
     op_t* stage = (op_t*)(smem + L::stage) + wave * L::PTS * in_stride(KS_IN);
     load_bias(net, bias, bias_lds);
+    const ChunkMasks cm = chunk_masks(net);
+    const bool wraps = ring_stream_path<HID_SOFTPLUS>() && ring_can_wrap(net);
+    RingStream rs = {0, false};
+    TileInputs<L::TILE> in(xc, worklist, 0, count, lane < L::PTS ? wave * L::PTS + lane : -1, blockIdx.x, gridDim.x);
     for (int t = blockIdx.x; t * L::TILE < count; t += gridDim.x) {
-        MP_STAMP_AT(HID_SOFTPLUS, 120, 0);
-        prologue_issue<KS_IN, WAVES>(net, wpack, smem + L::ring, wave, lane);
-        const int w = t * L::TILE + wave * L::PTS + lane;
-        const int id = (lane < L::PTS && w < count) ? (worklist ? worklist[w] : w) : -1;
-        if (lane < L::PTS) {
-            float x[3] = {0.f, 0.f, 0.f};
-            if (id >= 0) { x[0] = xc[3 * (size_t)id]; x[1] = xc[3 * (size_t)id + 1]; x[2] = xc[3 * (size_t)id + 2]; }
-            stage_pe<3, 6, KS_IN>(stage + lane * in_stride(KS_IN), x);
-        }
-        MP_STAMP_AT(HID_SOFTPLUS, 120, 1);
+        MP_STAMP_AT(HID_SOFTPLUS, 120 + MP_TILE_SLOT(t), 0);
+        const bool more = wraps && (long long)(t + gridDim.x) * L::TILE < count;
+        stream_prologue_issue<KS_IN, WAVES>(rs, net, wpack, smem + L::ring, wave, lane);
+        float x[3];
+        const int id = in.take(t, x);
+        if (lane < L::PTS) stage_pe<3, 6, KS_IN>(stage + lane * in_stride(KS_IN), x);
+        MP_STAMP_AT(HID_SOFTPLUS, 120 + MP_TILE_SLOT(t), 1);
         opx8 Bcur[KS_REG][NB];
         f32x4 out[NB];
         zero_b<NB>(Bcur);
-        prologue_wait();
-        MP_STAMP_AT(HID_SOFTPLUS, 120, 2);
-        run_net<NB, false, KS_IN, HID_SOFTPLUS, WAVES>(net, wpack, bias_lds, smem + L::ring, Bcur, stage, out, wave, lane);
-        MP_STAMP_AT(HID_SOFTPLUS, 120, 3);
+        stream_prologue_wait(rs);
+        MP_STAMP_AT(HID_SOFTPLUS, 120 + MP_TILE_SLOT(t), 2);
+        run_net<NB, false, KS_IN, HID_SOFTPLUS, WAVES>(net, wpack, bias_lds, smem + L::ring, Bcur, stage, out, wave, lane,
+                                                       SigIO{nullptr, 0}, NoCapture(), rs, cm, more ? wpack : nullptr, cm);
+        MP_STAMP_AT(HID_SOFTPLUS, 120 + MP_TILE_SLOT(t), 3);
 #pragma unroll
         for (int nb = 0; nb < NB; ++nb) {
             const int pid = __shfl(id, nb * 16 + (lane & 15));
             if (lane < 16 && pid >= 0) sdf_out[pid] = out[nb][0];
         }
-        MP_STAMP_AT(HID_SOFTPLUS, 121, 0);
+        MP_STAMP_AT(HID_SOFTPLUS, 121 + MP_TILE_SLOT(t), 0);
     }
 }
 
@@ -132,8 +169,12 @@
     float* bias_lds = (float*)(smem + L::bias0);
     op_t* stage = (op_t*)(smem + L::stage) + wave * L::PTS * STR;
     load_bias(net, bias, bias_lds);
+    const ChunkMasks cm = chunk_masks(net);
+    const bool wraps = ring_stream_path<HID_SOFTPLUS_X2>() && ring_can_wrap(net);
+    RingStream rs = {0, false};
     for (int t = blockIdx.x; t * TILE < count; t += gridDim.x) {
-        prologue_issue<KS_IN, WAVES>(net, wpack, smem + L::ring, wave, lane);
+        const bool more = wraps && (long long)(t + gridDim.x) * TILE < count;
+        stream_prologue_issue<KS_IN, WAVES>(rs, net, wpack, smem + L::ring, wave, lane);
         const int w = t * TILE + wave * WPTS + j;
         const int id = w < count ? (worklist ? worklist[w] : w) : -1;
         {
@@ -162,8 +203,9 @@
         opx8 Bcur[KS_REG][NB];
         f32x4 out[NB];
         zero_b<NB>(Bcur);
-        prologue_wait();
-        run_net<NB, false, KS_IN, HID_SOFTPLUS_X2, WAVES>(net, wpack, bias_lds, smem + L::ring, Bcur, stage, out, wave, lane);
+        stream_prologue_wait(rs);
+        run_net<NB, false, KS_IN, HID_SOFTPLUS_X2, WAVES>(net, wpack, bias_lds, smem + L::ring, Bcur, stage, out, wave, lane,
+                                                          SigIO{nullptr, 0}, NoCapture(), rs, cm, more ? wpack : nullptr, cm);
         if (lane < 16 && id >= 0) sdf_out[id] = out[0][0] + out[1][0];
     }
 }
@@ -316,28 +358,31 @@
     op_t* stage = (op_t*)(smem + L::stage) + wave * L::PTS * in_stride(KS_IN);
     load_bias(net, bias, bias_lds);
     constexpr int SIG_LAYER = KS_REG * SIG_CHUNK_BYTES;
+    const ChunkMasks cm = chunk_masks(net);
+    const bool wraps = ring_stream_path<HID_SOFTPLUS_SAVE>() && ring_can_wrap(net);
+    RingStream rs = {0, false};
+    TileInputs<L::TILE> in(xc, worklist, offset, count, lane < L::PTS ? wave * L::PTS + lane : -1, blockIdx.x, gridDim.x);
     for (int t = blockIdx.x; offset + t * L::TILE < count; t += gridDim.x) {
-        prologue_issue<KS_IN, WAVES>(net, wpack, smem + L::ring, wave, lane);
-        const int w = offset + t * L::TILE + wave * L::PTS + lane;
-        const int id = (lane < L::PTS && w < count) ? (worklist ? worklist[w] : w) : -1;
-        if (lane < L::PTS) {
-            float x[3] = {0.f, 0.f, 0.f};
-            if (id >= 0) { x[0] = xc[3 * (size_t)id]; x[1] = xc[3 * (size_t)id + 1]; x[2] = xc[3 * (size_t)id + 2]; }
-            stage_pe<3, 6, KS_IN>(stage + lane * in_stride(KS_IN), x);
-        }
+        MP_STAMP_AT(HID_SOFTPLUS_SAVE, 120 + MP_TILE_SLOT(t), 0);
+        const bool more = wraps && (long long)offset + (long long)(t + gridDim.x) * L::TILE < count;
+        stream_prologue_issue<KS_IN, WAVES>(rs, net, wpack, smem + L::ring, wave, lane);
+        float x[3];
+        const int id = in.take(t, x);
+        if (lane < L::PTS) stage_pe<3, 6, KS_IN>(stage + lane * in_stride(KS_IN), x);
+        MP_STAMP_AT(HID_SOFTPLUS_SAVE, 120 + MP_TILE_SLOT(t), 1);
         opx8 Bcur[KS_REG][NB];
         f32x4 out[NB];
         zero_b<NB>(Bcur);
-        prologue_wait();
-        MP_STAMP_AT(HID_SOFTPLUS_SAVE, 120, 2);
+        stream_prologue_wait(rs);
+        MP_STAMP_AT(HID_SOFTPLUS_SAVE, 120 + MP_TILE_SLOT(t), 2);
         #ifdef MP_EXP_SIGCACHED
         const SigIO sio = {sigbuf + ((size_t)(blockIdx.x) * WAVES + wave) * (size_t)(8 * SIG_LAYER), SIG_LAYER};
 #else
         const SigIO sio = {sigbuf + ((size_t)t * WAVES + wave) * (size_t)(8 * SIG_LAYER), SIG_LAYER};
 #endif
         run_net<NB, false, KS_IN, HID_SOFTPLUS_SAVE, WAVES>(net, wpack, bias_lds, smem + L::ring, Bcur, stage, out, wave, lane,
-                                                            sio);
-        MP_STAMP_AT(HID_SOFTPLUS_SAVE, 120, 3);
+                                                            sio, NoCapture(), rs, cm, more ? wpack : nullptr, cm);
+        MP_STAMP_AT(HID_SOFTPLUS_SAVE, 120 + MP_TILE_SLOT(t), 3);
         const size_t tile = (size_t)(offset / 64) + (size_t)t * 4 + (wave >> 1);
 #pragma unroll
         for (int nb = 0; nb < NB; ++nb) {
@@ -347,6 +392,7 @@
             const int pid = __shfl(id, nb * 16 + (lane & 15));
             if (lane < 16 && pid >= 0) sdf_out[pid] = out[nb][0];
         }
+        MP_STAMP_AT(HID_SOFTPLUS_SAVE, 121 + MP_TILE_SLOT(t), 0);
     }
 }
 
@@ -368,12 +414,22 @@
     op_t* tabs = w8 + 256 + wave * (2 * PTS * 48);
     for (int i = threadIdx.x; i < 256; i += blockDim.x) w8[i] = w8_slots[i];
     constexpr int SIG_LAYER = KS_REG * SIG_CHUNK_BYTES;
+    const ChunkMasks cm = chunk_masks(net);
+    const bool wraps = ring_stream_path<HID_SIGMUL>() && ring_can_wrap(net);
+    RingStream rs = {0, false};
+    TileInputs<TILE> in(xc, worklist, offset, count, wave * PTS + (lane & (PTS - 1)), blockIdx.x, gridDim.x);
+    __syncthreads();
     for (int t = blockIdx.x; offset + t * TILE < count; t += gridDim.x) {
-        const int w = offset + t * TILE + wave * PTS + (lane & (PTS - 1));
-        const int id = w < count ? (worklist ? worklist[w] : w) : -1;
+        MP_STAMP_AT(HID_SIGMUL, 120 + MP_TILE_SLOT(t), 0);
+        const bool more = wraps && (long long)offset + (long long)(t + gridDim.x) * TILE < count;
+#ifdef MP_EXP_GRAD_OLD
+        stream_prologue_issue<KS_IN, WAVES, false>(rs, net, wpack, smem, wave, lane);
+#else
+        stream_prologue_issue<KS_IN, WAVES>(rs, net, wpack, smem, wave, lane);
+#endif
+        float x[3];
+        const int id = in.take(t, x);
         if (lane < PTS) {
-            float x[3] = {0.f, 0.f, 0.f};
-            if (id >= 0) { x[0] = xc[3 * (size_t)id]; x[1] = xc[3 * (size_t)id + 1]; x[2] = xc[3 * (size_t)id + 2]; }
             op_t* ta = tabs + lane * 48;
             op_t* tb = tabs + PTS * 48 + lane * 48;
 #pragma unroll
@@ -400,7 +456,6 @@
         const SigIO sio = {const_cast<char*>(sigbuf) + ((size_t)t * WAVES + wave) * (size_t)(8 * SIG_LAYER), SIG_LAYER};
 #endif
         opx8 Bcur[KS_REG][NB];
-        __syncthreads();
 #pragma unroll
         for (int ks = 0; ks < KS_REG; ++ks) {
             const opx8 wv = *(const opx8*)(w8 + ks * 32 + 8 * gq);
@@ -425,15 +480,13 @@
         }
         float g[2][3] = {{0.f, 0.f, 0.f}, {0.f, 0.f, 0.f}};
         f32x4 out[NB];
-#ifdef MP_EXP_GRAD_OLD
-        prologue<KS_IN, WAVES, false>(net, wpack, smem, wave, lane);
-#else
-        prologue<KS_IN, WAVES>(net, wpack, smem, wave, lane);
-#endif
-        MP_STAMP_AT(HID_SIGMUL, 120, 2);
+        MP_STAMP_AT(HID_SIGMUL, 120 + MP_TILE_SLOT(t), 1);
+        stream_prologue_wait(rs);
+        MP_STAMP_AT(HID_SIGMUL, 120 + MP_TILE_SLOT(t), 2);
         run_net<NB, false, KS_IN, HID_SIGMUL, WAVES, GradCapture>(net, wpack, nullptr, smem, Bcur, nullptr, out, wave, lane, sio,
-                                                                   GradCapture{tabs, tabs + PTS * 48, g});
-        MP_STAMP_AT(HID_SIGMUL, 120, 3);
+                                                                   GradCapture{tabs, tabs + PTS * 48, g}, rs, cm,
+                                                                   more ? wpack : nullptr, cm);
+        MP_STAMP_AT(HID_SIGMUL, 120 + MP_TILE_SLOT(t), 3);
         GradCapture::unrotate(g);
 #pragma unroll
         for (int nb = 0; nb < NB; ++nb)
@@ -460,7 +513,7 @@
                 normal_out[3 * (size_t)pid + 2] = n2 * inv + poison;
             }
         }
-        __syncthreads();
+        MP_STAMP_AT(HID_SIGMUL, 121 + MP_TILE_SLOT(t), 0);
     }
 }
 
@@ -481,13 +534,18 @@
     float* bias_lds = (float*)(smem + L::bias0);
     op_t* stage = (op_t*)(smem + L::stage) + wave * L::PTS * in_stride(KS_IN);
     load_bias(net, bias, bias_lds);
+    const ChunkMasks cm = chunk_masks(net);
+    const bool wraps = ring_stream_path<HID_RELU>() && ring_can_wrap(net);
+    RingStream rs = {0, false};
+    TileInputs<L::TILE> in(xc, worklist, 0, count, lane < L::PTS ? wave * L::PTS + lane : -1, blockIdx.x, gridDim.x);
     for (int t = blockIdx.x; t * L::TILE < count; t += gridDim.x) {
-        MP_STAMP_AT(HID_RELU, 120, 0);
+        MP_STAMP_AT(HID_RELU, 120 + MP_TILE_SLOT(t), 0);
+        const bool more = wraps && (long long)(t + gridDim.x) * L::TILE < count;
         const int w0 = t * L::TILE + wave * L::PTS;
         const int tile = w0 / 64, nb0 = (w0 % 64) / 16;
-        const int w = w0 + lane;
-        const int id = (lane < L::PTS && w < count) ? (worklist ? worklist[w] : w) : -1;
-        prologue_issue<KS_IN, WAVES>(net, wpack, smem + L::ring, wave, lane);
+        float x[3];
+        const int id = in.take(t, x);
+        stream_prologue_issue<KS_IN, WAVES>(rs, net, wpack, smem + L::ring, wave, lane);
         opx8 Bcur[KS_REG][NB];
         const bool live = w0 < count;
 #pragma unroll
@@ -503,17 +561,18 @@
             if (id >= 0) {
 #pragma unroll
                 for (int a = 0; a < 3; ++a) {
-                    row[a] = (op_t)xc[3 * (size_t)id + a];
+                    row[a] = (op_t)x[a];
                     row[3 + a] = (op_t)normal[3 * (size_t)id + a];
                 }
             }
         }
-        MP_STAMP_AT(HID_RELU, 120, 1);
+        MP_STAMP_AT(HID_RELU, 120 + MP_TILE_SLOT(t), 1);
         f32x4 out[NB];
-        prologue_wait();
-        MP_STAMP_AT(HID_RELU, 120, 2);
-        run_net<NB, false, KS_IN, HID_RELU, WAVES>(net, wpack, bias_lds, smem + L::ring, Bcur, stage, out, wave, lane);
-        MP_STAMP_AT(HID_RELU, 120, 3);
+        stream_prologue_wait(rs);
+        MP_STAMP_AT(HID_RELU, 120 + MP_TILE_SLOT(t), 2);
+        run_net<NB, false, KS_IN, HID_RELU, WAVES>(net, wpack, bias_lds, smem + L::ring, Bcur, stage, out, wave, lane,
+                                                   SigIO{nullptr, 0}, NoCapture(), rs, cm, more ? wpack : nullptr, cm);
+        MP_STAMP_AT(HID_RELU, 120 + MP_TILE_SLOT(t), 3);
 #pragma unroll
         for (int nb = 0; nb < NB; ++nb) {
             const int pid = __shfl(id, nb * 16 + (lane & 15));
@@ -524,7 +583,7 @@
                 for (int c = 0; c < 3; ++c) rgb_out[3 * (size_t)pid + c] = 1.0f / (1.0f + __expf(-out[nb][c])) + poison;
             }
         }
-        MP_STAMP_AT(HID_RELU, 121, 0);
+        MP_STAMP_AT(HID_RELU, 121 + MP_TILE_SLOT(t), 0);
     }
 }
 
@@ -538,7 +597,7 @@
                                                            float radius, float* __restrict__ bg_rgb) {
     constexpr int KS_IN = 3, NBG = 32;
     using L = Lds<KS_IN, NB, WAVES>;
-    static_assert(L::PTS % NBG == 0, "whole rays per wave");
+    static_assert(L::PTS == NBG, "one ray per wave");
     extern __shared__ __attribute__((aligned(16))) char smem[];
     const int wave = threadIdx.x >> 6, lane = threadIdx.x & 63;
     float* bias_lds0 = (float*)(smem + L::bias0);
@@ -549,8 +608,12 @@
     load_bias(net_ren, bias_ren, bias_lds1);
     const int n_pts = n_rays * NBG;
     const float ox = cam[0], oy = cam[1], oz = cam[2];
+    const ChunkMasks cm_imp = chunk_masks(net_imp), cm_ren = chunk_masks(net_ren);
+    const bool wraps = ring_stream_path<HID_SOFTPLUS>() && ring_can_wrap(net_imp) && ring_can_wrap(net_ren);
+    RingStream rs = {0, false};
     for (int t = blockIdx.x; t * L::TILE < n_pts; t += gridDim.x) {
-        prologue_issue<KS_IN, WAVES>(net_imp, wp_imp, smem + L::ring, wave, lane);
+        const bool more = wraps && (long long)(t + gridDim.x) * L::TILE < n_pts;
+        stream_prologue_issue<KS_IN, WAVES>(rs, net_imp, wp_imp, smem + L::ring, wave, lane);
         const int q = t * L::TILE + wave * L::PTS + lane;
         const int ray = q / NBG, s = q % NBG;
         float d[3] = {0.f, 0.f, 1.f};
@@ -585,41 +648,52 @@
         opx8 Bcur[KS_REG][NB];
         f32x4 out[NB];
         zero_b<NB>(Bcur);
-        prologue_wait();
+        stream_prologue_wait(rs);
         run_net<NB, false, KS_IN, HID_SOFTPLUS, WAVES>(net_imp, wp_imp, bias_lds0, smem + L::ring, Bcur, stage, out, wave,
-                                                       lane);
-        prologue_issue<KS_IN, WAVES>(net_ren, wp_ren, smem + L::ring, wave, lane);
+                                                       lane, SigIO{nullptr, 0}, NoCapture(), rs, cm_imp, wraps ? wp_ren : nullptr, cm_ren);
+        stream_prologue_issue<KS_IN, WAVES>(rs, net_ren, wp_ren, smem + L::ring, wave, lane);
         if (lane < 16) {
 #pragma unroll
             for (int nb = 0; nb < NB; ++nb) scr[(nb * 16 + lane) * 4 + 3] = fabsf(out[nb][0]);
         }
         if (lane < L::PTS) stage_pe<3, 4, KS_IN>(stage + lane * in_stride(KS_IN), d);
-        prologue_wait();
-        run_net<NB, false, KS_IN, HID_RELU, WAVES>(net_ren, wp_ren, bias_lds1, smem + L::ring, Bcur, stage, out, wave, lane);
+        stream_prologue_wait(rs);
+        run_net<NB, false, KS_IN, HID_RELU, WAVES>(net_ren, wp_ren, bias_lds1, smem + L::ring, Bcur, stage, out, wave, lane,
+                                                   SigIO{nullptr, 0}, NoCapture(), rs, cm_ren, more ? wp_imp : nullptr, cm_imp);
         if (lane < 16) {
 #pragma unroll
             for (int nb = 0; nb < NB; ++nb)
 #pragma unroll
                 for (int c = 0; c < 3; ++c) scr[(nb * 16 + lane) * 4 + c] = 1.0f / (1.0f + __expf(-out[nb][c]));
         }
-        __syncthreads();
-        if (lane < L::PTS / NBG) {
-            const int r = (t * L::TILE + wave * L::PTS) / NBG + lane;
-            if (r < n_rays) {
-                float acc[3] = {0.f, 0.f, 0.f}, csum = 0.0f;
-                for (int i = 0; i < NBG; ++i) {
-                    const float zi = z_per_ray ? z_bg[(size_t)r * NBG + i] : z_bg[i];
-                    const float zn = i + 1 < NBG ? (z_per_ray ? z_bg[(size_t)r * NBG + i + 1] : z_bg[i + 1]) : 0.f;
-                    const float dist = i + 1 < NBG ? zi - zn : 1e10f;
-                    const float* sp = scr + (lane * NBG + i) * 4;
-                    const float fe = dist * sp[3];
-                    const float alpha = 1.0f - expf(-fe);
-                    const float wgt = alpha * expf(-csum);
-                    acc[0] += wgt * sp[0]; acc[1] += wgt * sp[1]; acc[2] += wgt * sp[2];
-                    csum += fe;
-                }
-                bg_rgb[3 * r] = acc[0]; bg_rgb[3 * r + 1] = acc[1]; bg_rgb[3 * r + 2] = acc[2];
-            }
+        const int r = (t * L::TILE + wave * L::PTS) / NBG;
+        if (r < n_rays) {
+            float dist = 0.0f, dens = 0.0f, alpha = 0.0f, col[3] = {0.f, 0.f, 0.f};
+            if (lane < NBG) {
+                const int i = lane;
+                const float zi = z_per_ray ? z_bg[(size_t)r * NBG + i] : z_bg[i];
+                const float zn = i + 1 < NBG ? (z_per_ray ? z_bg[(size_t)r * NBG + i + 1] : z_bg[i + 1]) : 0.f;
+                dist = i + 1 < NBG ? zi - zn : 1e10f;
+                const float* sp = scr + i * 4;
+                dens = sp[3];
+                alpha = 1.0f - expf(-(dist * dens));
+                col[0] = sp[0]; col[1] = sp[1]; col[2] = sp[2];
+            }
+            float csum = 0.0f, before = 0.0f;
+#pragma unroll 2
+            for (int i = 0; i < NBG; ++i) {
+                before = lane == i ? csum : before;
+                csum = __builtin_fmaf(lane_value(dist, i), lane_value(dens, i), csum);
+            }
+            const float wgt = alpha * expf(-before);
+            float acc[3] = {0.f, 0.f, 0.f};
+#pragma unroll 2
+            for (int i = 0; i < NBG; ++i) {
+                const float wi = lane_value(wgt, i);
+#pragma unroll
+                for (int c = 0; c < 3; ++c) acc[c] = __builtin_fmaf(wi, lane_value(col[c], i), acc[c]);
+            }
+            if (lane == 0) { bg_rgb[3 * r] = acc[0]; bg_rgb[3 * r + 1] = acc[1]; bg_rgb[3 * r + 2] = acc[2]; }
         }
     }
 }
diff --git a/multiply_amd/csrc/mlp_core.hpp b/multiply_amd/csrc/mlp_core.hpp
--- a/multiply_amd/csrc/mlp_core.hpp
+++ b/multiply_amd/csrc/mlp_core.hpp
@@ -85,6 +85,7 @@
 #endif
 #define MP_STAMP_OK(hid) (MP_STAMP_HID < 0 || (hid) == MP_STAMP_HID)
 #define MP_STAMP(ev) do { if (MP_STAMP_OK(HID) && blockIdx.x == 0 && lane == 0 && ci < 120) mp_stamps[((wave) * 128 + ci) * 4 + (ev)] = __builtin_amdgcn_s_memtime(); } while (0)
+#define MP_TILE_SLOT(t) (2 * (((t) / (int)gridDim.x) & 1))
 #define MP_STAMP_AT(hid, slot, ev) do { if (MP_STAMP_OK(hid) && blockIdx.x == 0 && (threadIdx.x & 63) == 0) mp_stamps[((threadIdx.x >> 6) * 128 + (slot)) * 4 + (ev)] = __builtin_amdgcn_s_memtime(); } while (0)
 #else
 #define MP_STAMP(ev)
@@ -592,17 +593,37 @@
     }
 }
 
+template <int P>
+struct PartC { static constexpr int value = P; };
+
 struct NoCapture {
     template <int NB>
     __device__ __forceinline__ void operator()(int, int, const f32x4 (&)[NB]) const {}
 };
+
+struct RingStream {
+    int pos;
+    bool fed;
+};
+template <int HID>
+__host__ __device__ constexpr bool ring_stream_path() {
+#if defined(MP_EXP_NOPP)
+    return false;
+#elif defined(MP_EXP_GRAD_OLD)
+    return HID != HID_SIGMUL;
+#else
+    return true;
+#endif
+}
+__device__ __forceinline__ bool ring_can_wrap(const NetDesc& net) { return net.total_chunks >= RING_SLOTS; }
 
 template <int KS_IN, int HID, int WAVES, bool HIDDEN, typename Cap, typename NB_T>
 __device__ __forceinline__ void run_layer_pp(const NetDesc& net, const LayerDesc L, int l, const char* __restrict__ wpack,
                                              const float* bias_lds, char* wring, opx8 (&Bcur)[KS_REG][2], NB_T& Bn,
                                              opx8 (&aq)[AQ_LEN], u32x4 (&sgb)[SIG_BUFS][2], const op_t* stage_wave,
                                              f32x4 (&out)[2], int wave, int lane, const SigIO& sig, Cap& cap, int& ci,
-                                             int& ring_pos, const ChunkMasks& cm, const DmaLanes<KS_IN>& dl, int pp_last) {
+                                             int& ring_pos, const ChunkMasks& cm, const DmaLanes<KS_IN>& dl, int pp_last, bool fed,
+                                             const char* __restrict__ next_wpack, const ChunkMasks& next_cm) {
     constexpr int PF = PP_PF, QN = PP_QN, NT = 2 * KS_REG;
     constexpr bool BIAS = HID != HID_SIGMUL;
     const int g = lane >> 4;
@@ -611,6 +632,15 @@
     const int cap_id = (L.aux >> 8) & 0xff;
     const bool late = __builtin_amdgcn_readfirstlane(wave) >= WAVES / 2;
     const ActConst kact = act_const();
+    auto issue_ahead = [&](auto part, int ahead, int slot) {
+        const int cn = ci + ahead;
+        const bool wrap = cn > pp_last;
+        if (!wrap || next_wpack != nullptr) {
+            const ChunkMasks m = {{wrap ? next_cm.reg[0] : cm.reg[0], wrap ? next_cm.reg[1] : cm.reg[1]},
+                                  {wrap ? next_cm.in[0] : cm.in[0], wrap ? next_cm.in[1] : cm.in[1]}};
+            pp_issue<KS_IN, decltype(part)::value>(wrap ? next_wpack : wpack, wring, wrap ? cn - pp_last - 1 : cn, slot, m, dl);
+        }
+    };
 #pragma unroll
     for (int c = 0; c < MAX_CHUNKS; ++c) {
         if ((HIDDEN ? c < KS_REG : true) && c < L.n_chunk) {
@@ -707,14 +737,14 @@
 #if defined(MP_DMA_SPLIT)
                 if constexpr (!REV) dma_wait_all();
                 __syncthreads();
-                if (ci + 3 <= pp_last) pp_issue<KS_IN, 2>(wpack, wring, ci + 3, ring_pos, cm, dl);
+                issue_ahead(PartC<2>{}, 3, ring_pos);
 #elif defined(MP_DMA_EARLY)
                 __syncthreads();
 #else
                 if constexpr (!REV) dma_wait_all();
                 __syncthreads();
 #ifndef MP_EXP_NOLOAD
-                if (ci + 3 <= pp_last) pp_issue<KS_IN>(wpack, wring, ci + 3, ring_pos, cm, dl);
+                issue_ahead(PartC<0>{}, 3, ring_pos);
 #endif
 #endif
                 MP_STAMP(2);
@@ -751,11 +781,9 @@
                 else if constexpr (!REV) dma_wait_all();
 #ifndef MP_EXP_NOLOAD
 #ifdef MP_DMA_SPLIT
-                if (ci >= 1 && ci + 2 <= pp_last)
-                    pp_issue<KS_IN, 1>(wpack, wring, ci + 2, ring_pos == 0 ? RING_SLOTS - 1 : ring_pos - 1, cm, dl);
-#else
-                if (ci >= 1 && ci + 2 <= pp_last)
-                    pp_issue<KS_IN>(wpack, wring, ci + 2, ring_pos == 0 ? RING_SLOTS - 1 : ring_pos - 1, cm, dl);
+                if (ci >= 1 || fed) issue_ahead(PartC<1>{}, 2, ring_pos == 0 ? RING_SLOTS - 1 : ring_pos - 1);
+#else
+                if (ci >= 1 || fed) issue_ahead(PartC<0>{}, 2, ring_pos == 0 ? RING_SLOTS - 1 : ring_pos - 1);
 #endif
 #endif
 #endif
@@ -936,8 +964,8 @@
 template <int NB, bool FWD, int KS_IN, int HID, int WAVES, typename Cap = NoCapture>
 __device__ __forceinline__ void run_net(const NetDesc& net, const char* __restrict__ wpack, const float* bias_lds,
                                         char* wring, opx8 (&Bcur)[KS_REG][NB], const op_t* stage_wave,
-                                        f32x4 (&out)[NB], int wave, int lane, SigIO sig = SigIO{nullptr, 0},
-                                        Cap cap = Cap()) {
+                                        f32x4 (&out)[NB], int wave, int lane, SigIO sig, Cap cap, RingStream& rs,
+                                        const ChunkMasks& cm, const char* __restrict__ next_wpack, const ChunkMasks& next_cm) {
     int ci = 0;
     u32x4 sgb[SIG_BUFS][NB];
 #pragma unroll
@@ -963,18 +991,20 @@
                   "the interleaved (round-1) stream stores half-precision sigmoids: build the ablation with -DMP_EXP_SIG16");
     if constexpr (PP) {
         const int pp_last = net.total_chunks - 1;
-        const ChunkMasks cm = chunk_masks(net);
         const DmaLanes<KS_IN> dl = dma_lanes<KS_IN>(__builtin_amdgcn_readfirstlane(wave) & (WAVES / 2 - 1), lane);
-        int ring_pos = 0;
+        int ring_pos = rs.pos;
+        const bool fed = rs.fed;
 #pragma unroll
         for (int t = 0; t < PP_PF; ++t)
-            aq[t % PP_QN] = *(const opx8*)(wring + (t % 2) * mb_bytes(KS_IN) + (t / 2) * TILE_BYTES + lane * 16);
+            aq[t % PP_QN] = *(const opx8*)(wring + ring_pos * chunk_bytes(KS_IN) + (t % 2) * mb_bytes(KS_IN) + (t / 2) * TILE_BYTES + lane * 16);
         for (; l < net.n_layers && net.layer[l].act != ACT_NONE; ++l)
             run_layer_pp<KS_IN, HID, WAVES, true>(net, net.layer[l], l, wpack, bias_lds, wring, Bcur, Bn, aq, sgb, stage_wave, out,
-                                                  wave, lane, sig, cap, ci, ring_pos, cm, dl, pp_last);
+                                                  wave, lane, sig, cap, ci, ring_pos, cm, dl, pp_last, fed, next_wpack, next_cm);
         for (; l < net.n_layers; ++l)
             run_layer_pp<KS_IN, HID, WAVES, false>(net, net.layer[l], l, wpack, bias_lds, wring, Bcur, Bn, aq, sgb, stage_wave, out,
-                                                   wave, lane, sig, cap, ci, ring_pos, cm, dl, pp_last);
+                                                   wave, lane, sig, cap, ci, ring_pos, cm, dl, pp_last, fed, next_wpack, next_cm);
+        rs.pos = next_wpack != nullptr ? ring_pos : 0;
+        rs.fed = next_wpack != nullptr;
     }
     if constexpr (!PP) {
         for (; l < net.n_layers && net.layer[l].act != ACT_NONE; ++l)
@@ -984,6 +1014,16 @@
     for (; l < net.n_layers; ++l)
         run_layer<NB, FWD, KS_IN, HID, WAVES, false>(net, net.layer[l], l, wpack, bias_lds, wring, Bcur, Bn, aq, sgb, stage_wave,
                                                      out, wave, lane, sig, cap, ci);
+}
+
+template <int NB, bool FWD, int KS_IN, int HID, int WAVES, typename Cap = NoCapture>
+__device__ __forceinline__ void run_net(const NetDesc& net, const char* __restrict__ wpack, const float* bias_lds,
+                                        char* wring, opx8 (&Bcur)[KS_REG][NB], const op_t* stage_wave,
+                                        f32x4 (&out)[NB], int wave, int lane, SigIO sig = SigIO{nullptr, 0},
+                                        Cap cap = Cap()) {
+    RingStream rs = {0, false};
+    const ChunkMasks cm = chunk_masks(net);
+    run_net<NB, FWD, KS_IN, HID, WAVES, Cap>(net, wpack, bias_lds, wring, Bcur, stage_wave, out, wave, lane, sig, cap, rs, cm, nullptr, cm);
 }
 
 #ifdef MP_EXP_NOPP
@@ -1009,6 +1049,14 @@
     prologue_issue<KS_IN, WAVES, THREE>(net, wpack, wring, wave, lane);
     prologue_wait();
 }
+template <int KS_IN, int WAVES, bool THREE = PROLOGUE_THREE>
+__device__ __forceinline__ void stream_prologue_issue(const RingStream& rs, const NetDesc& net, const char* __restrict__ wpack,
+                                                      char* wring, int wave, int lane) {
+    if (!rs.fed) prologue_issue<KS_IN, WAVES, THREE>(net, wpack, wring, wave, lane);
+}
+__device__ __forceinline__ void stream_prologue_wait(const RingStream& rs) {
+    if (!rs.fed) prologue_wait();
+}
 __device__ __forceinline__ void load_bias(const NetDesc& net, const float* __restrict__ bias, float* bias_lds) {
     for (int i = threadIdx.x; i < net.n_layers * BIAS_STRIDE; i += blockDim.x) bias_lds[i] = bias[i];
 }
```

Result: faster. 2.903 million rays/s, median of 6 (+1.7%).
